# spcl/gemm_hls

Measured on NVIDIA H100. Metric: GFLOP/s at N=16384 K=16384 M=16384 float (Multiply,Add), higher is better.
Workload: dtype tf32 tensor-core multiply, f32 accumulate/storage

## Files before the change

### gemm_hls_b200/csrc/capi.cu

```cuda
#include <algorithm>
#include <chrono>
#include <condition_variable>
#include <cstdlib>
#include <cstring>
#include <functional>
#include <mutex>
#include <string>
#include <thread>
#include <vector>

#include "common.cuh"

namespace mm {

namespace {
thread_local std::string g_last_error = "";
}

void set_error(const std::string &msg) { g_last_error = msg; }
int fail(int code, const std::string &msg) {
  set_error(msg);
  return code;
}

namespace {

struct KnobInfo {
  const char *env;
  int dflt;
};
const KnobInfo kKnobs[MM_TUNE_COUNT] = {
    {"MM_TCGEN05_CTA_GROUP", 2}, {"MM_TCGEN05_BLOCK_N", 256},  {"MM_TCGEN05_STAGES", 0},
    {"MM_TCGEN05_RASTER_ROWS", 2048}, {"MM_TCGEN05_TILE_SYNC", 1}, {"MM_TCGEN05_B_MN", 1},
    {"MM_TCGEN05_L2", 0}, {"MM_TCGEN05_B_OVERLAP", 0}, {"MM_TCGEN05_TMA_STORE", 1},
    {"MM_DMMA_TILE_ROWS", 0}, {"MM_EXPERIMENT_TF32_NO_ROUND", 0}, {"MM_SEMIRING_RING", 1},
};

}

int tuning_validate(int knob, int value) {
  bool ok = false;
  switch (knob) {
    case MM_TUNE_TCGEN05_CTA_GROUP: ok = value == 1 || value == 2; break;
    case MM_TUNE_TCGEN05_BLOCK_N: ok = value == 128 || value == 256; break;
    case MM_TUNE_TCGEN05_STAGES: ok = value == 0 || (value >= 2 && value <= 8); break;
    case MM_TUNE_TCGEN05_RASTER_ROWS: ok = value >= 1; break;
    case MM_TUNE_TCGEN05_L2_POLICY: ok = value >= 0 && value <= 2; break;
    case MM_TUNE_DMMA_TILE_ROWS: ok = value == 0 || value == 64 || value == 128; break;
    case MM_TUNE_TCGEN05_TILE_SYNC:
    case MM_TUNE_TCGEN05_B_MN:
    case MM_TUNE_TCGEN05_B_OVERLAP:
    case MM_TUNE_TCGEN05_TMA_STORE:
    case MM_TUNE_EXPERIMENT_TF32_NO_ROUND:
    case MM_TUNE_SEMIRING_RING: ok = value == 0 || value == 1; break;
    default: return fail(MM_ERR_INVALID, "unknown tuning knob " + std::to_string(knob));
  }
  if (!ok) {
    return fail(MM_ERR_INVALID, std::string("value ") + std::to_string(value) + " is out of range for tuning knob " +
                                    kKnobs[knob].env);
  }
  return MM_OK;
}

Tuning default_tuning() {
  Tuning t;
  for (int i = 0; i < MM_TUNE_COUNT; ++i) {
    t.v[i] = kKnobs[i].dflt;
    const char *e = std::getenv(kKnobs[i].env);
    if (!e || !*e) continue;
    int value;
    if (i == MM_TUNE_TCGEN05_L2_POLICY && (e[0] == 'n' || e[0] == 'f' || e[0] == 'l')) {
      value = e[0] == 'f' ? 1 : (e[0] == 'l' ? 2 : 0);
    } else {
      value = std::atoi(e);
    }
    if (tuning_validate(i, value) == MM_OK) t.v[i] = value;
  }
  return t;
}

}

struct mm_context {
  int device = 0;
  cudaStream_t stream = nullptr;
  cudaStream_t side = nullptr;
  cudaStream_t copy_in = nullptr, copy_out = nullptr;
  std::vector<cudaEvent_t> sync_events;
  cudaEvent_t ev_start = nullptr, ev_stop = nullptr, ev_fork = nullptr, ev_join = nullptr;
  cudaEvent_t ev_slice = nullptr;
  mm::Scratch scratch;
  mm::Scratch staging[3];
  uint64_t staging_gen = 0;
  std::vector<void *> retired;
  bool captured = false;
  mm::Tuning tuning;
  bool profiling = false;
  std::vector<cudaEvent_t> prof_events;
  int prof_calls = 0;
  std::mutex mutex;
};

namespace {

using mm::fail;

bool valid_dtype(int d) { return d >= 0 && d < MM_DTYPE_COUNT; }
bool valid_op(int o) { return o >= 0 && o < MM_OP_COUNT; }

enum Path { kPathTcgen05, kPathDmma, kPathSemiring };

bool tensor_core_dtype(int d) {
  return d == MM_DTYPE_FLOAT || d == MM_DTYPE_HALF || d == MM_DTYPE_BFLOAT16 || d == MM_DTYPE_UINT8;
}

constexpr unsigned kMaxKInt8Tensor = 33024;

Path select_path(int dtype, int map_op, int reduce_op, int flags, unsigned n, unsigned k) {
  const bool dense = (map_op == MM_OP_MULTIPLY && reduce_op == MM_OP_ADD) && !(flags & MM_FLAG_EXACT);
  if (dense && (dtype == MM_DTYPE_FLOAT || dtype == MM_DTYPE_HALF || dtype == MM_DTYPE_BFLOAT16)) return kPathTcgen05;
  if (dense && dtype == MM_DTYPE_UINT8 && k <= kMaxKInt8Tensor) return kPathTcgen05;
  if (dense && dtype == MM_DTYPE_DOUBLE) {
    return ((flags & MM_FLAG_TRANSPOSED_A) && (n % 2 != 0)) ? kPathSemiring : kPathDmma;
  }
  return kPathSemiring;
}

int ensure(mm_context *ctx, mm::Scratch &s, size_t bytes, bool keep_old) {
  if (s.bytes >= bytes) return MM_OK;
  if (s.ptr) {
    if (keep_old) ctx->retired.push_back(s.ptr);
    else cudaFree(s.ptr);
  }
  s.ptr = nullptr;
  s.bytes = 0;
  cudaError_t e = cudaMalloc(&s.ptr, bytes);
  if (e != cudaSuccess) {
    return fail(e == cudaErrorMemoryAllocation ? MM_ERR_NOMEM : MM_ERR_CUDA,
                std::string("cudaMalloc(") + std::to_string(bytes) + "): " + cudaGetErrorString(e));
  }
  s.bytes = bytes;
  return MM_OK;
}

int check_args(int dtype, int map_op, int reduce_op, const void *a, const void *b, const void *c,
               unsigned n, unsigned k, unsigned m) {
  if (!valid_dtype(dtype)) return fail(MM_ERR_INVALID, "unknown MM_DATA_TYPE code");
  if (!valid_op(map_op) || !valid_op(reduce_op)) return fail(MM_ERR_INVALID, "unknown MM_MAP_OP / MM_REDUCE_OP code");
  if (!a || !b || !c) return fail(MM_ERR_INVALID, "null matrix pointer");
  if (n == 0 || k == 0 || m == 0) return fail(MM_ERR_INVALID, "matrix dimensions must be positive");
  const unsigned w = mm_memory_width(dtype);
  if (k % w != 0) {
    return fail(MM_ERR_SHAPE, "K (" + std::to_string(k) + ") must be divisable by the memory width in K (" +
                                  std::to_string(w) + ").");
  }
  if (m % w != 0) {
    return fail(MM_ERR_SHAPE, "M (" + std::to_string(m) + ") must be divisable by the memory width in M (" +
                                  std::to_string(w) + ").");
  }
  return MM_OK;
}

int check_device_alignment(const void *a, const void *b, const void *c) {
  if ((reinterpret_cast<uintptr_t>(a) | reinterpret_cast<uintptr_t>(b) | reinterpret_cast<uintptr_t>(c)) % 16 != 0) {
    return fail(MM_ERR_INVALID, "device matrix pointers must be 16-byte aligned");
  }
  return MM_OK;
}

mm::GemmArgs make_args(mm_context *ctx, const void *a, const void *b, void *c, unsigned n, unsigned k, unsigned m,
                       int flags, cudaStream_t stream) {
  mm::GemmArgs g{a, b, c, n, k, m, flags, stream};
  g.tuning = &ctx->tuning;
  g.side_stream = ctx->side;
  g.ev_fork = ctx->ev_fork;
  g.ev_join = ctx->ev_join;
  return g;
}

mm::GemmBatch make_batch(unsigned batch, int flags) {
  mm::GemmBatch bt;
  bt.count = batch;
  bt.shared_a = (flags & MM_FLAG_BATCH_SHARED_A) != 0;
  bt.shared_b = (flags & MM_FLAG_BATCH_SHARED_B) != 0;
  return bt;
}

int check_batch(unsigned batch, unsigned n, unsigned k, unsigned m) {
  if (batch == 0) return fail(MM_ERR_INVALID, "batch must be positive");
  if (batch > 65535) {
    return fail(MM_ERR_UNSUPPORTED, "batch (" + std::to_string(batch) + ") must not exceed 65535");
  }
  const uint64_t limit = uint64_t(1) << 31;
  if (uint64_t(batch) * n >= limit || uint64_t(batch) * k >= limit || uint64_t(batch) * m >= limit) {
    return fail(MM_ERR_UNSUPPORTED, "batch * N, batch * K and batch * M must be below 2^31");
  }
  return MM_OK;
}

bool overlaps(const void *x, size_t x_bytes, const void *y, size_t y_bytes) {
  const uintptr_t x0 = reinterpret_cast<uintptr_t>(x), y0 = reinterpret_cast<uintptr_t>(y);
  return x0 < y0 + y_bytes && y0 < x0 + x_bytes;
}

int begin_call(mm_context *ctx, cudaStream_t stream, bool profile, cudaStreamCaptureStatus *capture,
               cudaEvent_t **pe) {
  *capture = cudaStreamCaptureStatusNone;
  if (cudaStreamIsCapturing(stream, capture) == cudaSuccess && *capture != cudaStreamCaptureStatusNone) {
    ctx->captured = true;
  }
  *pe = nullptr;
  if (profile && ctx->profiling && ctx->prof_calls < 256) {
    while (ctx->prof_events.size() < size_t(3 * (ctx->prof_calls + 1))) {
      cudaEvent_t e;
      MM_CUDA_TRY(cudaEventCreate(&e));
      ctx->prof_events.push_back(e);
    }
    *pe = &ctx->prof_events[3 * ctx->prof_calls];
    ++ctx->prof_calls;
    MM_CUDA_TRY(cudaEventRecord((*pe)[0], stream));
  }
  return MM_OK;
}

int enqueue_locked(mm_context *ctx, int dtype, int map_op, int reduce_op, int flags, const void *a,
                   const void *b, void *c, unsigned n, unsigned k, unsigned m, cudaStream_t stream,
                   bool dry_run = false, unsigned batch = 1, bool accumulate = false,
                   const mm::AgreeFn *agree = nullptr) {
  mm::GemmArgs g = make_args(ctx, a, b, c, n, k, m, flags, stream);
  g.agree = agree;
  g.batch = make_batch(batch, flags);
  g.dry_run = dry_run;
  g.accumulate = accumulate;
  cudaStreamCaptureStatus capture;
  cudaEvent_t *pe;
  const int rc_begin = begin_call(ctx, stream, !dry_run, &capture, &pe);
  if (rc_begin != MM_OK) return rc_begin;
  if (pe) {
    g.ev_start = pe[0];
    g.ev_prep_done = pe[1];
  }
  int rc_launch = MM_OK;
  switch (select_path(dtype, map_op, reduce_op, flags, n, k)) {
    case kPathTcgen05: {
      const size_t need = mm::tcgen05_scratch_bytes(dtype, n, k, m, flags, ctx->tuning, g.batch);
      if (need > ctx->scratch.bytes && capture != cudaStreamCaptureStatusNone) {
        return fail(MM_ERR_INVALID, batch > 1 ? "the scratch cannot grow during stream capture: call mm_context_reserve_batched() first"
                                              : "the scratch cannot grow during stream capture: call mm_context_reserve() first");
      }
      int rc = ensure(ctx, ctx->scratch, need, ctx->captured);
      if (rc != MM_OK) return rc;
      rc_launch = mm::launch_tcgen05(dtype, g, ctx->scratch.ptr, ctx->scratch.bytes);
      break;
    }
    case kPathDmma:
      if (pe) MM_CUDA_TRY(cudaEventRecord(pe[1], stream));
      rc_launch = accumulate ? mm::launch_dmma_accumulate(g) : mm::launch_dmma(g);
      break;
    case kPathSemiring:
      if (pe) MM_CUDA_TRY(cudaEventRecord(pe[1], stream));
      rc_launch = accumulate ? mm::launch_semiring_accumulate(dtype, map_op, reduce_op, g)
                             : mm::launch_semiring(dtype, map_op, reduce_op, g);
      break;
  }
  if (rc_launch != MM_OK) return rc_launch;
  if (pe) MM_CUDA_TRY(cudaEventRecord(pe[2], stream));
  return MM_OK;
}

void destroy_context(mm_context *ctx) {
  cudaSetDevice(ctx->device);
  if (ctx->stream) cudaStreamSynchronize(ctx->stream);
  if (ctx->side) cudaStreamSynchronize(ctx->side);
  if (ctx->scratch.ptr) cudaFree(ctx->scratch.ptr);
  for (auto &s : ctx->staging) {
    if (s.ptr) cudaFree(s.ptr);
  }
  for (void *p : ctx->retired) cudaFree(p);
  for (auto e : ctx->prof_events) cudaEventDestroy(e);
  for (auto e : ctx->sync_events) cudaEventDestroy(e);
  for (cudaEvent_t e : {ctx->ev_start, ctx->ev_stop, ctx->ev_fork, ctx->ev_join, ctx->ev_slice}) {
    if (e) cudaEventDestroy(e);
  }
  for (cudaStream_t s : {ctx->copy_in, ctx->copy_out, ctx->side, ctx->stream}) {
    if (s) cudaStreamDestroy(s);
  }
  delete ctx;
}

int init_context(mm_context *ctx) {
  MM_CUDA_TRY(cudaStreamCreateWithFlags(&ctx->stream, cudaStreamNonBlocking));
  MM_CUDA_TRY(cudaStreamCreateWithFlags(&ctx->side, cudaStreamNonBlocking));
  MM_CUDA_TRY(cudaStreamCreateWithFlags(&ctx->copy_in, cudaStreamNonBlocking));
  MM_CUDA_TRY(cudaStreamCreateWithFlags(&ctx->copy_out, cudaStreamNonBlocking));
  MM_CUDA_TRY(cudaEventCreate(&ctx->ev_start));
  MM_CUDA_TRY(cudaEventCreate(&ctx->ev_stop));
  MM_CUDA_TRY(cudaEventCreateWithFlags(&ctx->ev_fork, cudaEventDisableTiming));
  MM_CUDA_TRY(cudaEventCreateWithFlags(&ctx->ev_join, cudaEventDisableTiming));
  MM_CUDA_TRY(cudaEventCreateWithFlags(&ctx->ev_slice, cudaEventDisableTiming));
  return MM_OK;
}

struct BPlan {
  unsigned k0 = 0, k1 = 0;
  const void *const *parts_dev = nullptr;
  unsigned parts = 1, part_rows = 0;
  std::vector<cudaEvent_t> peer_slices;
};

struct Pipeline {
  mm_context *ctx;
  int dtype, map_op, reduce_op, flags;
  const unsigned char *a_host;
  const unsigned char *b_host;
  unsigned char *c_host;
  unsigned rows, k, m;
  size_t es;
  Path path;
  unsigned char *da = nullptr, *db = nullptr, *dc = nullptr;

  int upload_b(const BPlan &bp) {
    MM_CUDA_TRY(cudaSetDevice(ctx->device));
    ++ctx->staging_gen;
    int rc;
    if ((rc = ensure(ctx, ctx->staging[0], size_t(rows) * k * es, false)) != MM_OK) return rc;
    if ((rc = ensure(ctx, ctx->staging[1], size_t(k) * m * es, false)) != MM_OK) return rc;
    if ((rc = ensure(ctx, ctx->staging[2], size_t(rows) * m * es, false)) != MM_OK) return rc;
    if (path == kPathTcgen05) {
      rc = ensure(ctx, ctx->scratch, mm::tcgen05_scratch_bytes(dtype, rows, k, m, flags, ctx->tuning), ctx->captured);
      if (rc != MM_OK) return rc;
    }
    da = static_cast<unsigned char *>(ctx->staging[0].ptr);
    db = static_cast<unsigned char *>(ctx->staging[1].ptr);
    dc = static_cast<unsigned char *>(ctx->staging[2].ptr);
    const size_t off = size_t(bp.k0) * m * es, bytes = size_t(bp.k1 - bp.k0) * m * es;
    if (bytes) MM_CUDA_TRY(cudaMemcpyAsync(db + off, b_host + off, bytes, cudaMemcpyHostToDevice, ctx->copy_in));
    MM_CUDA_TRY(cudaEventRecord(ctx->ev_slice, ctx->copy_in));
    return MM_OK;
  }

  int run(const BPlan &bp, double *seconds_device, const mm::AgreeFn *agree = nullptr) {
    const int rc = enqueue_all(bp, agree);
    cudaError_t e = cudaSuccess;
    for (cudaStream_t s : {ctx->copy_in, ctx->side, ctx->stream, ctx->copy_out}) {
      const cudaError_t es_ = cudaStreamSynchronize(s);
      if (e == cudaSuccess) e = es_;
    }
    if (rc != MM_OK) return rc;
    if (e != cudaSuccess) return fail(MM_ERR_CUDA, std::string("host pipeline: ") + cudaGetErrorString(e));
    if (seconds_device) {
      float ms = 0.f;
      MM_CUDA_TRY(cudaEventElapsedTime(&ms, ctx->ev_start, ctx->ev_stop));
      *seconds_device = 1e-3 * ms;
    }
    return MM_OK;
  }

 private:
  int enqueue_all(const BPlan &bp, const mm::AgreeFn *agree) {
    MM_CUDA_TRY(cudaSetDevice(ctx->device));
    const bool ta = (flags & MM_FLAG_TRANSPOSED_A) != 0;
    const mm::Tuning &t = ctx->tuning;
    unsigned chunk_rows = rows;
    if (!ta) {
      const size_t row_bytes = size_t(k) * es;
      size_t cr = std::max<size_t>((rows + 15) / 16, ((size_t(32) << 20) + row_bytes - 1) / row_bytes);
      if (const char *e = std::getenv("MM_HOST_CHUNK_ROWS")) cr = std::max(1, std::atoi(e));
      cr = (cr + 127) / 128 * 128;
      if (cr < rows) chunk_rows = unsigned(cr);
    }
    const unsigned chunks = (rows + chunk_rows - 1) / chunk_rows;
    while (ctx->sync_events.size() < size_t(2 * chunks)) {
      cudaEvent_t e;
      MM_CUDA_TRY(cudaEventCreateWithFlags(&e, cudaEventDisableTiming));
      ctx->sync_events.push_back(e);
    }
    auto ev_a = [&](unsigned i) { return ctx->sync_events[i]; };
    auto ev_c = [&](unsigned i) { return ctx->sync_events[chunks + i]; };

    for (unsigned i = 0; i < chunks; ++i) {
      const size_t r0 = size_t(i) * chunk_rows, nr = std::min<size_t>(chunk_rows, rows - r0);
      if (!ta) {
        MM_CUDA_TRY(cudaMemcpyAsync(da + r0 * k * es, a_host + r0 * k * es, nr * k * es, cudaMemcpyHostToDevice,
                                    ctx->copy_in));
      } else {
        MM_CUDA_TRY(cudaMemcpyAsync(da, a_host, size_t(rows) * k * es, cudaMemcpyHostToDevice, ctx->copy_in));
      }
      MM_CUDA_TRY(cudaEventRecord(ev_a(i), ctx->copy_in));
    }

    MM_CUDA_TRY(cudaStreamWaitEvent(ctx->stream, ctx->ev_slice, 0));
    for (cudaEvent_t e : bp.peer_slices) MM_CUDA_TRY(cudaStreamWaitEvent(ctx->stream, e, 0));
    MM_CUDA_TRY(cudaEventRecord(ctx->ev_start, ctx->stream));
    mm::BSource src;
    src.b = db;
    if (bp.parts_dev != nullptr) {
      src.src = bp.parts_dev;
      src.parts = bp.parts;
      src.part_rows = bp.part_rows;
    }
    int rc = MM_OK;
    mm::PreparedB pb;
    unsigned char *aprep = nullptr;
    mm::HalfScratch hs;
    if (path == kPathTcgen05) {
      hs = mm::tcgen05_half_scratch(ctx->scratch.ptr, ctx->scratch.bytes, dtype, rows, k, m, flags, t);
      if (hs.fits_b) MM_CUDA_TRY(cudaMemsetAsync(hs.fits_b, 1, hs.flag_bytes, ctx->stream));
      rc = mm::tcgen05_prepare_b_async(dtype, src, db, ctx->scratch.ptr, ctx->scratch.bytes, k, m, flags, t, ctx->stream,
                                       ctx->side, ctx->ev_fork, ctx->ev_join, &pb, 1, hs.b, hs.fits_b);
      if (rc != MM_OK) return rc;
      aprep = static_cast<unsigned char *>(ctx->scratch.ptr) + mm::tcgen05_bt_bytes(dtype, k, m, flags, t);
    } else if (bp.parts_dev != nullptr) {
      rc = mm::gather_b_rows(src, db, es, k, m, ctx->stream);
      if (rc != MM_OK) return rc;
    }
    const bool prepare_first = hs.fits_a != nullptr;
    std::vector<const void *> a_ops(chunks);
    auto prepare = [&](unsigned i) -> int {
      const size_t r0 = size_t(i) * chunk_rows, nr = std::min<size_t>(chunk_rows, rows - r0);
      MM_CUDA_TRY(cudaStreamWaitEvent(ctx->stream, ev_a(i), 0));
      if (path != kPathTcgen05) return MM_OK;
      const size_t a_scale = (dtype == MM_DTYPE_FLOAT && (flags & MM_FLAG_TF32X3)) ? 3 : 1;
      return mm::tcgen05_prepare_a(dtype, da + (ta ? 0 : r0 * k * es), aprep + (ta ? 0 : r0 * k * es * a_scale),
                                   unsigned(nr), k, flags, t, &a_ops[i], ctx->stream, 1,
                                   hs.a ? static_cast<unsigned char *>(hs.a) + r0 * k * 2 : nullptr, hs.fits_a);
    };
    auto compute = [&](unsigned i) -> int {
      const size_t r0 = size_t(i) * chunk_rows, nr = std::min<size_t>(chunk_rows, rows - r0);
      const void *a_chunk = da + (ta ? 0 : r0 * k * es);
      void *c_chunk = dc + r0 * m * es;
      int rc1;
      if (path == kPathTcgen05) {
        mm::HalfOperands half = hs.operands();
        if (half.a) half.a = static_cast<const unsigned char *>(half.a) + r0 * k * 2;
        const mm::Tcgen05Counters cnt = mm::tcgen05_counters(ctx->scratch.ptr, ctx->scratch.bytes);
        rc1 = mm::tcgen05_gemm(dtype, a_ops[i], pb.b_op, c_chunk, unsigned(nr), k, m, flags, t, cnt.tile_sync, pb.ready,
                               pb.ready_target, ctx->stream, mm::GemmBatch{}, false, half);
      } else {
        mm::GemmArgs g = make_args(ctx, a_chunk, db, c_chunk, unsigned(nr), k, m, flags, ctx->stream);
        rc1 = (path == kPathDmma) ? mm::launch_dmma(g) : mm::launch_semiring(dtype, map_op, reduce_op, g);
      }
      if (rc1 == MM_OK) MM_CUDA_TRY(cudaEventRecord(ev_c(i), ctx->stream));
      return rc1;
    };
    if (prepare_first) {
      for (unsigned i = 0; i < chunks && rc == MM_OK; ++i) rc = prepare(i);
    }
    if (rc == MM_OK && agree != nullptr) rc = (*agree)(hs.fits_a, ctx->stream);
    for (unsigned i = 0; i < chunks && rc == MM_OK; ++i) {
      if (!prepare_first) rc = prepare(i);
      if (rc == MM_OK) rc = compute(i);
    }
    if (path == kPathTcgen05 && pb.forked) cudaStreamWaitEvent(ctx->stream, ctx->ev_join, 0);
    if (rc != MM_OK) return rc;
    MM_CUDA_TRY(cudaEventRecord(ctx->ev_stop, ctx->stream));

    for (unsigned i = 0; i < chunks; ++i) {
      const size_t r0 = size_t(i) * chunk_rows, nr = std::min<size_t>(chunk_rows, rows - r0);
      MM_CUDA_TRY(cudaStreamWaitEvent(ctx->copy_out, ev_c(i), 0));
      MM_CUDA_TRY(cudaMemcpyAsync(c_host + r0 * m * es, dc + r0 * m * es, nr * m * es, cudaMemcpyDeviceToHost,
                                  ctx->copy_out));
    }
    return MM_OK;
  }
};

std::mutex g_default_mutex;
mm_context *g_default_ctx = nullptr;
mm_multi *g_default_multi = nullptr;

int env_int(const char *name, int fallback) {
  const char *e = std::getenv(name);
  return (e && *e) ? std::atoi(e) : fallback;
}

class HostBarrier {
 public:
  explicit HostBarrier(int n) : n_(n) {}
  void arrive_and_wait() {
    std::unique_lock<std::mutex> lock(m_);
    const int gen = gen_;
    if (++count_ == n_) {
      count_ = 0;
      ++gen_;
      cv_.notify_all();
    } else {
      cv_.wait(lock, [&] { return gen_ != gen; });
    }
  }

 private:
  std::mutex m_;
  std::condition_variable cv_;
  int n_, count_ = 0, gen_ = 0;
};

class FitsAgreement {
 public:
  FitsAgreement(HostBarrier &barrier, int gpus) : barrier_(barrier), fit_(gpus, 1), agreed_(gpus, 0) {}
  mm::AgreeFn agree(int g) {
    return [this, g](unsigned int *fits, cudaStream_t stream) -> int {
      agreed_[g] = 1;
      int rc = MM_OK;
      unsigned int v = 1;
      if (fits != nullptr) {
        cudaError_t e = cudaStreamSynchronize(stream);
        if (e == cudaSuccess) e = cudaMemcpy(&v, fits, sizeof(v), cudaMemcpyDeviceToHost);
        if (e != cudaSuccess) rc = fail(MM_ERR_CUDA, std::string("reading the fits word of A: ") + cudaGetErrorString(e));
      }
      fit_[g] = v != 0u;
      barrier_.arrive_and_wait();
      const bool all = std::all_of(fit_.begin(), fit_.end(), [](int f) { return f != 0; });
      if (rc == MM_OK && fits != nullptr && v != 0u && !all) MM_CUDA_TRY(cudaMemsetAsync(fits, 0, sizeof(v), stream));
      return rc;
    };
  }
  void finish(int g) {
    if (!agreed_[g]) barrier_.arrive_and_wait();
  }

 private:
  HostBarrier &barrier_;
  std::vector<int> fit_;
  std::vector<char> agreed_;
};

}

struct mm_multi {
  std::vector<mm_context *> ctx;
  std::vector<void **> parts_dev;
  bool peer = false;
  std::mutex mutex;
  unsigned n = 0, k = 0, m = 0;
  int dtype = -1;
  std::vector<uint64_t> gen;
  bool executed = false;
};

namespace {

unsigned rows_per_gpu(unsigned n, int g) { return (n + unsigned(g) - 1) / unsigned(g); }

struct Partition {
  unsigned r0, r1;
  unsigned k0, k1;
  unsigned part_rows, parts;
};
Partition partition_for(int gpus, int g, unsigned n, unsigned k, bool sliced_b) {
  Partition p;
  const unsigned per = rows_per_gpu(n, gpus);
  p.r0 = std::min(n, unsigned(g) * per);
  p.r1 = std::min(n, p.r0 + per);
  p.part_rows = sliced_b ? std::max(64u, (rows_per_gpu(k, gpus) + 63u) / 64u * 64u) : k;
  p.parts = sliced_b ? (k + p.part_rows - 1) / p.part_rows : 1;
  if (sliced_b) {
    p.k0 = std::min(k, unsigned(g) * p.part_rows);
    p.k1 = (unsigned(g) >= p.parts) ? p.k0 : std::min(k, p.k0 + p.part_rows);
  } else {
    p.k0 = 0;
    p.k1 = k;
  }
  return p;
}

template <class Fn>
int fan_out(int gpus, Fn fn) {
  std::vector<int> rc(gpus, MM_OK);
  std::vector<std::string> msg(gpus);
  std::vector<std::thread> pool;
  for (int g = 0; g < gpus; ++g) {
    pool.emplace_back([&, g] {
      rc[g] = fn(g);
      if (rc[g] != MM_OK) msg[g] = mm_last_error();
    });
  }
  for (auto &t : pool) t.join();
  for (int g = 0; g < gpus; ++g) {
    if (rc[g] != MM_OK) return fail(rc[g], "GPU " + std::to_string(g) + ": " + msg[g]);
  }
  return MM_OK;
}

int refresh_parts(mm_multi *mu, int g) {
  mm_context *ctx = mu->ctx[g];
  MM_CUDA_TRY(cudaSetDevice(ctx->device));
  std::vector<void *> table(mu->ctx.size());
  for (size_t j = 0; j < mu->ctx.size(); ++j) table[j] = mu->ctx[j]->staging[1].ptr;
  MM_CUDA_TRY(cudaMemcpy(mu->parts_dev[g], table.data(), table.size() * sizeof(void *), cudaMemcpyHostToDevice));
  return MM_OK;
}

int multi_gemm_host_locked(mm_multi *mu, int dtype, int map_op, int reduce_op, int flags, const void *a, const void *b,
                           void *c, unsigned n, unsigned k, unsigned m, double *seconds_device) {
  if (flags & MM_FLAG_TRANSPOSED_A) {
    return fail(MM_ERR_UNSUPPORTED, "the row-block split over GPUs needs row-major A (MM_TRANSPOSED_A is set)");
  }
  const int G = int(mu->ctx.size());
  const size_t es = mm_dtype_size(dtype);
  std::vector<Pipeline> pipes(G);
  std::vector<BPlan> plans(G);
  std::vector<double> dev_s(G, 0.0);
  HostBarrier barrier(G);
  FitsAgreement fits(barrier, G);
  int rc = fan_out(G, [&](int g) -> int {
    const Partition part = partition_for(G, g, n, k, mu->peer);
    const unsigned r0 = part.r0, r1 = part.r1;
    Pipeline &p = pipes[g];
    p = Pipeline{mu->ctx[g], dtype, map_op, reduce_op, flags,
                 static_cast<const unsigned char *>(a) + size_t(r0) * k * es, static_cast<const unsigned char *>(b),
                 static_cast<unsigned char *>(c) + size_t(r0) * m * es, r1 - r0, k, m, es,
                 select_path(dtype, map_op, reduce_op, flags, std::max(1u, r1 - r0), k)};
    BPlan &bp = plans[g];
    bp.k0 = part.k0;
    bp.k1 = part.k1;
    if (mu->peer) {
      bp.parts = part.parts;
      bp.part_rows = part.part_rows;
      bp.parts_dev = mu->parts_dev[g];
    }
    std::lock_guard<std::mutex> lock(mu->ctx[g]->mutex);
    if (p.rows == 0) p.rows = 1, p.a_host = static_cast<const unsigned char *>(a), p.c_host = nullptr;
    int rc1 = p.upload_b(bp);
    barrier.arrive_and_wait();
    int rc2 = (rc1 == MM_OK && mu->peer) ? refresh_parts(mu, g) : MM_OK;
    if (mu->peer) {
      for (int j = 0; j < G; ++j) {
        if (j != g) bp.peer_slices.push_back(mu->ctx[j]->ev_slice);
      }
    }
    barrier.arrive_and_wait();
    const mm::AgreeFn agree = fits.agree(g);
    int rc3 = MM_OK;
    if (rc1 == MM_OK && rc2 == MM_OK && r1 > r0) {
      rc3 = p.run(bp, &dev_s[g], &agree);
    } else {
      cudaSetDevice(mu->ctx[g]->device);
      cudaStreamSynchronize(mu->ctx[g]->copy_in);
    }
    fits.finish(g);
    barrier.arrive_and_wait();
    return rc1 != MM_OK ? rc1 : (rc2 != MM_OK ? rc2 : rc3);
  });
  if (rc != MM_OK) return rc;
  if (seconds_device) *seconds_device = *std::max_element(dev_s.begin(), dev_s.end());
  return MM_OK;
}

void clear_resident(mm_multi *mu) {
  mu->n = mu->k = mu->m = 0;
  mu->dtype = -1;
  mu->gen.clear();
  mu->executed = false;
}

int check_resident(mm_multi *mu, const char *entry, int dtype, unsigned n, unsigned k, unsigned m) {
  if (mu->dtype != dtype || mu->n != n || mu->k != k || mu->m != m) {
    return fail(MM_ERR_INVALID, std::string(entry) + ": no matching mm_multi_upload (type or sizes differ)");
  }
  for (size_t g = 0; g < mu->ctx.size(); ++g) {
    std::lock_guard<std::mutex> lock(mu->ctx[g]->mutex);
    if (mu->ctx[g]->staging_gen != mu->gen[g]) {
      return fail(MM_ERR_INVALID, std::string(entry) + ": no matching mm_multi_upload (GPU " + std::to_string(g) +
                                      "'s buffers were reused by another call since)");
    }
  }
  return MM_OK;
}

int create_multi(int n_gpus, const int *devices, mm_multi **out) {
  mm_multi *mu = new mm_multi();
  auto cleanup = [&](int rc) {
    const std::string msg = mm_last_error();
    mm_multi_destroy(mu);
    mm::set_error(msg);
    return rc;
  };
  for (int g = 0; g < n_gpus; ++g) {
    mm_context *c = nullptr;
    const int rc = mm_context_create(devices ? devices[g] : g, &c);
    if (rc != MM_OK) return cleanup(rc);
    mu->ctx.push_back(c);
  }
  mu->peer = n_gpus > 1;
  for (int g = 0; g < n_gpus && mu->peer; ++g) {
    for (int j = 0; j < n_gpus; ++j) {
      if (mu->ctx[j]->device == mu->ctx[g]->device) continue;
      int can = 0;
      if (cudaDeviceCanAccessPeer(&can, mu->ctx[g]->device, mu->ctx[j]->device) != cudaSuccess || !can) mu->peer = false;
    }
  }
  for (int g = 0; g < n_gpus; ++g) {
    if (cudaSetDevice(mu->ctx[g]->device) != cudaSuccess) return cleanup(fail(MM_ERR_CUDA, "cudaSetDevice failed"));
    for (int j = 0; j < n_gpus && mu->peer; ++j) {
      if (mu->ctx[j]->device == mu->ctx[g]->device) continue;
      const cudaError_t e = cudaDeviceEnablePeerAccess(mu->ctx[j]->device, 0);
      if (e == cudaErrorPeerAccessAlreadyEnabled) cudaGetLastError();
      else if (e != cudaSuccess) mu->peer = false;
    }
    void **table = nullptr;
    if (cudaMalloc(&table, sizeof(void *) * size_t(n_gpus)) != cudaSuccess) {
      return cleanup(fail(MM_ERR_NOMEM, "cudaMalloc of the slice table failed"));
    }
    mu->parts_dev.push_back(table);
  }
  *out = mu;
  return MM_OK;
}

int kernel_execute(mm_context *ctx, int dtype, int map_op, int reduce_op, int flags, const void *a, const void *b,
                   void *c, unsigned n, unsigned k, unsigned m, double *seconds_device, double *seconds_wall,
                   const mm::AgreeFn *agree) {
  if (!ctx) return fail(MM_ERR_INVALID, "null context");
  int rc = check_args(dtype, map_op, reduce_op, a, b, c, n, k, m);
  if (rc != MM_OK) return rc;
  if ((rc = check_device_alignment(a, b, c)) != MM_OK) return rc;
  std::lock_guard<std::mutex> lock(ctx->mutex);
  MM_CUDA_TRY(cudaSetDevice(ctx->device));
  rc = enqueue_locked(ctx, dtype, map_op, reduce_op, flags, a, b, c, n, k, m, ctx->stream, true);
  if (rc != MM_OK) return rc;
  const auto t0 = std::chrono::high_resolution_clock::now();
  MM_CUDA_TRY(cudaEventRecord(ctx->ev_start, ctx->stream));
  rc = enqueue_locked(ctx, dtype, map_op, reduce_op, flags, a, b, c, n, k, m, ctx->stream, false, 1, false, agree);
  if (rc != MM_OK) {
    cudaStreamSynchronize(ctx->stream);
    return rc;
  }
  MM_CUDA_TRY(cudaEventRecord(ctx->ev_stop, ctx->stream));
  MM_CUDA_TRY(cudaEventSynchronize(ctx->ev_stop));
  const auto t1 = std::chrono::high_resolution_clock::now();
  float ms = 0.f;
  MM_CUDA_TRY(cudaEventElapsedTime(&ms, ctx->ev_start, ctx->ev_stop));
  if (seconds_device) *seconds_device = 1e-3 * ms;
  if (seconds_wall) *seconds_wall = std::chrono::duration<double>(t1 - t0).count();
  return MM_OK;
}

}

extern "C" {

const char *mm_last_error(void) { return mm::g_last_error.c_str(); }

int mm_version(void) { return 203; }

size_t mm_dtype_size(int dtype) {
  switch (dtype) {
    case MM_DTYPE_HALF: return 2;
    case MM_DTYPE_FLOAT: return 4;
    case MM_DTYPE_DOUBLE: return 8;
    case MM_DTYPE_INT32: return 4;
    case MM_DTYPE_UINT32: return 4;
    case MM_DTYPE_UINT8: return 1;
    case MM_DTYPE_BFLOAT16: return 2;
  }
  return 0;
}

unsigned mm_memory_width(int dtype) {
  const size_t s = mm_dtype_size(dtype);
  return s ? static_cast<unsigned>(64 / s) : 0;
}

int mm_context_create(int device, mm_context **out) {
  if (!out) return fail(MM_ERR_INVALID, "null output pointer");
  *out = nullptr;
  int count = 0;
  cudaError_t e = cudaGetDeviceCount(&count);
  if (e != cudaSuccess || count == 0) {
    return fail(MM_ERR_CUDA, std::string("no CUDA device available: ") +
                                 (e != cudaSuccess ? cudaGetErrorString(e) : "device count is 0"));
  }
  if (device < 0 || device >= count) return fail(MM_ERR_INVALID, "device ordinal out of range");
  MM_CUDA_TRY(cudaSetDevice(device));
  cudaDeviceProp prop;
  MM_CUDA_TRY(cudaGetDeviceProperties(&prop, device));
  if (prop.major != 9 || prop.minor != 0) {
    return fail(MM_ERR_UNSUPPORTED, std::string("libmm_b200 is built for sm_90a only; device is sm_") +
                                        std::to_string(prop.major) + std::to_string(prop.minor));
  }
  mm_context *ctx = new mm_context();
  ctx->device = device;
  ctx->tuning = mm::default_tuning();
  const int rc = init_context(ctx);
  if (rc != MM_OK) {
    const std::string msg = mm_last_error();
    destroy_context(ctx);
    mm::set_error(msg);
    return rc;
  }
  *out = ctx;
  return MM_OK;
}

int mm_context_destroy(mm_context *ctx) {
  if (!ctx) return MM_OK;
  destroy_context(ctx);
  return MM_OK;
}

int mm_context_set_tuning(mm_context *ctx, int knob, int value) {
  if (!ctx) return fail(MM_ERR_INVALID, "null context");
  const int rc = mm::tuning_validate(knob, value);
  if (rc != MM_OK) return rc;
  std::lock_guard<std::mutex> lock(ctx->mutex);
  ctx->tuning.v[knob] = value;
  return MM_OK;
}

int mm_context_get_tuning(mm_context *ctx, int knob, int *value) {
  if (!ctx || !value) return fail(MM_ERR_INVALID, "null argument");
  if (knob < 0 || knob >= MM_TUNE_COUNT) return fail(MM_ERR_INVALID, "unknown tuning knob " + std::to_string(knob));
  std::lock_guard<std::mutex> lock(ctx->mutex);
  *value = ctx->tuning.v[knob];
  return MM_OK;
}

int mm_context_reserve(mm_context *ctx, int dtype, int flags, unsigned n, unsigned k, unsigned m) {
  if (!ctx) return fail(MM_ERR_INVALID, "null context");
  if (!valid_dtype(dtype)) return fail(MM_ERR_INVALID, "unknown MM_DATA_TYPE code");
  std::lock_guard<std::mutex> lock(ctx->mutex);
  MM_CUDA_TRY(cudaSetDevice(ctx->device));
  if (!tensor_core_dtype(dtype)) return MM_OK;
  return ensure(ctx, ctx->scratch, mm::tcgen05_scratch_bytes(dtype, n, k, m, flags & ~MM_FLAG_EXACT, ctx->tuning),
                ctx->captured);
}

int mm_context_reserve_batched(mm_context *ctx, int dtype, int flags, unsigned n, unsigned k, unsigned m,
                               unsigned batch) {
  if (!ctx) return fail(MM_ERR_INVALID, "null context");
  if (!valid_dtype(dtype)) return fail(MM_ERR_INVALID, "unknown MM_DATA_TYPE code");
  int rc = check_batch(batch, n, k, m);
  if (rc != MM_OK) return rc;
  std::lock_guard<std::mutex> lock(ctx->mutex);
  MM_CUDA_TRY(cudaSetDevice(ctx->device));
  if (!tensor_core_dtype(dtype)) return MM_OK;
  const int f = flags & ~MM_FLAG_EXACT;
  return ensure(ctx, ctx->scratch, mm::tcgen05_scratch_bytes(dtype, n, k, m, f, ctx->tuning, make_batch(batch, f)),
                ctx->captured);
}

int mm_buffer_alloc(mm_context *ctx, size_t bytes, void **device_ptr) {
  if (!ctx || !device_ptr) return fail(MM_ERR_INVALID, "null argument");
  *device_ptr = nullptr;
  MM_CUDA_TRY(cudaSetDevice(ctx->device));
  cudaError_t e = cudaMalloc(device_ptr, bytes ? bytes : 1);
  if (e != cudaSuccess) {
    return fail(e == cudaErrorMemoryAllocation ? MM_ERR_NOMEM : MM_ERR_CUDA,
                std::string("cudaMalloc: ") + cudaGetErrorString(e));
  }
  return MM_OK;
}

int mm_buffer_free(mm_context *ctx, void *device_ptr) {
  if (!ctx) return fail(MM_ERR_INVALID, "null context");
  MM_CUDA_TRY(cudaSetDevice(ctx->device));
  MM_CUDA_TRY(cudaFree(device_ptr));
  return MM_OK;
}

int mm_copy_to_device(mm_context *ctx, void *device_dst, const void *host_src, size_t bytes) {
  if (!ctx || !device_dst || !host_src) return fail(MM_ERR_INVALID, "null argument");
  std::lock_guard<std::mutex> lock(ctx->mutex);
  MM_CUDA_TRY(cudaSetDevice(ctx->device));
  MM_CUDA_TRY(cudaMemcpyAsync(device_dst, host_src, bytes, cudaMemcpyHostToDevice, ctx->stream));
  MM_CUDA_TRY(cudaStreamSynchronize(ctx->stream));
  return MM_OK;
}

int mm_copy_to_host(mm_context *ctx, void *host_dst, const void *device_src, size_t bytes) {
  if (!ctx || !host_dst || !device_src) return fail(MM_ERR_INVALID, "null argument");
  std::lock_guard<std::mutex> lock(ctx->mutex);
  MM_CUDA_TRY(cudaSetDevice(ctx->device));
  MM_CUDA_TRY(cudaMemcpyAsync(host_dst, device_src, bytes, cudaMemcpyDeviceToHost, ctx->stream));
  MM_CUDA_TRY(cudaStreamSynchronize(ctx->stream));
  return MM_OK;
}

int mm_kernel_enqueue(mm_context *ctx, int dtype, int map_op, int reduce_op, int flags,
                      const void *a, const void *b, void *c, unsigned n, unsigned k, unsigned m,
                      void *cuda_stream) {
  if (!ctx) return fail(MM_ERR_INVALID, "null context");
  int rc = check_args(dtype, map_op, reduce_op, a, b, c, n, k, m);
  if (rc != MM_OK) return rc;
  if ((rc = check_device_alignment(a, b, c)) != MM_OK) return rc;
  std::lock_guard<std::mutex> lock(ctx->mutex);
  MM_CUDA_TRY(cudaSetDevice(ctx->device));
  cudaStream_t s = cuda_stream ? static_cast<cudaStream_t>(cuda_stream) : ctx->stream;
  return enqueue_locked(ctx, dtype, map_op, reduce_op, flags, a, b, c, n, k, m, s);
}

int mm_kernel_enqueue_batched(mm_context *ctx, int dtype, int map_op, int reduce_op, int flags, const void *a,
                              const void *b, void *c, unsigned n, unsigned k, unsigned m, unsigned batch,
                              void *cuda_stream) {
  if (!ctx) return fail(MM_ERR_INVALID, "null context");
  int rc = check_args(dtype, map_op, reduce_op, a, b, c, n, k, m);
  if (rc != MM_OK) return rc;
  if ((rc = check_batch(batch, n, k, m)) != MM_OK) return rc;
  if ((rc = check_device_alignment(a, b, c)) != MM_OK) return rc;
  std::lock_guard<std::mutex> lock(ctx->mutex);
  MM_CUDA_TRY(cudaSetDevice(ctx->device));
  cudaStream_t s = cuda_stream ? static_cast<cudaStream_t>(cuda_stream) : ctx->stream;
  return enqueue_locked(ctx, dtype, map_op, reduce_op, flags, a, b, c, n, k, m, s, false, batch);
}

int mm_kernel_enqueue_accumulate(mm_context *ctx, int dtype, int map_op, int reduce_op, int flags, const void *a,
                                 const void *b, void *c, unsigned n, unsigned k, unsigned m, unsigned batch,
                                 void *cuda_stream) {
  if (!ctx) return fail(MM_ERR_INVALID, "null context");
  int rc = check_args(dtype, map_op, reduce_op, a, b, c, n, k, m);
  if (rc != MM_OK) return rc;
  if ((rc = check_batch(batch, n, k, m)) != MM_OK) return rc;
  if ((rc = check_device_alignment(a, b, c)) != MM_OK) return rc;
  const size_t es = mm_dtype_size(dtype);
  const mm::GemmBatch bt = make_batch(batch, flags);
  if (overlaps(c, size_t(batch) * n * m * es, a, size_t(bt.a_copies()) * n * k * es) ||
      overlaps(c, size_t(batch) * n * m * es, b, size_t(bt.b_copies()) * k * m * es)) {
    return fail(MM_ERR_INVALID, "C must not overlap A or B in an accumulating call");
  }
  std::lock_guard<std::mutex> lock(ctx->mutex);
  MM_CUDA_TRY(cudaSetDevice(ctx->device));
  cudaStream_t s = cuda_stream ? static_cast<cudaStream_t>(cuda_stream) : ctx->stream;
  return enqueue_locked(ctx, dtype, map_op, reduce_op, flags, a, b, c, n, k, m, s, false, batch,
                        true);
}

int mm_kernel_enqueue_witness(mm_context *ctx, int dtype, int map_op, int reduce_op, int flags, const void *a,
                              const void *b, void *c, unsigned *w, unsigned n, unsigned k, unsigned m, unsigned batch,
                              void *cuda_stream) {
  if (!ctx) return fail(MM_ERR_INVALID, "null context");
  int rc = check_args(dtype, map_op, reduce_op, a, b, c, n, k, m);
  if (rc != MM_OK) return rc;
  if ((rc = check_batch(batch, n, k, m)) != MM_OK) return rc;
  if ((rc = check_device_alignment(a, b, c)) != MM_OK) return rc;
  if (!w) return fail(MM_ERR_INVALID, "null witness pointer");
  if (reinterpret_cast<uintptr_t>(w) % 16 != 0) return fail(MM_ERR_INVALID, "the witness pointer must be 16-byte aligned");
  if (reduce_op != MM_OP_MIN && reduce_op != MM_OP_MAX) {
    return fail(MM_ERR_INVALID, "witnesses exist for the Min and Max reduces only");
  }
  std::lock_guard<std::mutex> lock(ctx->mutex);
  MM_CUDA_TRY(cudaSetDevice(ctx->device));
  cudaStream_t s = cuda_stream ? static_cast<cudaStream_t>(cuda_stream) : ctx->stream;
  mm::GemmArgs g = make_args(ctx, a, b, c, n, k, m, flags, s);
  g.batch = make_batch(batch, flags);
  cudaStreamCaptureStatus capture;
  cudaEvent_t *pe;
  if ((rc = begin_call(ctx, s, true, &capture, &pe)) != MM_OK) return rc;
  if (pe) MM_CUDA_TRY(cudaEventRecord(pe[1], s));
  if ((rc = mm::launch_semiring_witness(dtype, map_op, reduce_op, g, w)) != MM_OK) return rc;
  if (pe) MM_CUDA_TRY(cudaEventRecord(pe[2], s));
  return MM_OK;
}

int mm_kernel_execute(mm_context *ctx, int dtype, int map_op, int reduce_op, int flags,
                      const void *a, const void *b, void *c, unsigned n, unsigned k, unsigned m,
                      double *seconds_device, double *seconds_wall) {
  return kernel_execute(ctx, dtype, map_op, reduce_op, flags, a, b, c, n, k, m, seconds_device, seconds_wall, nullptr);
}

int mm_context_set_profiling(mm_context *ctx, int enable) {
  if (!ctx) return fail(MM_ERR_INVALID, "null context");
  std::lock_guard<std::mutex> lock(ctx->mutex);
  ctx->profiling = enable != 0;
  ctx->prof_calls = 0;
  return MM_OK;
}

int mm_context_profile_read(mm_context *ctx, double *prep_sum, double *main_sum, int *calls) {
  if (!ctx) return fail(MM_ERR_INVALID, "null context");
  std::lock_guard<std::mutex> lock(ctx->mutex);
  MM_CUDA_TRY(cudaSetDevice(ctx->device));
  double prep = 0.0, main_s = 0.0;
  for (int i = 0; i < ctx->prof_calls; ++i) {
    cudaEvent_t *e = &ctx->prof_events[3 * i];
    MM_CUDA_TRY(cudaEventSynchronize(e[2]));
    float ms_prep = 0.f, ms_main = 0.f;
    MM_CUDA_TRY(cudaEventElapsedTime(&ms_prep, e[0], e[1]));
    MM_CUDA_TRY(cudaEventElapsedTime(&ms_main, e[1], e[2]));
    prep += 1e-3 * ms_prep;
    main_s += 1e-3 * ms_main;
  }
  if (prep_sum) *prep_sum = prep;
  if (main_sum) *main_sum = main_s;
  if (calls) *calls = ctx->prof_calls;
  ctx->prof_calls = 0;
  return MM_OK;
}

int mm_kernel_launch_count(int dtype, int map_op, int reduce_op, int flags) {
  if (!valid_dtype(dtype) || !valid_op(map_op) || !valid_op(reduce_op)) return -1;
  const mm::Tuning t = mm::default_tuning();
  switch (select_path(dtype, map_op, reduce_op, flags, 2, 64)) {
    case kPathTcgen05:
      return 1 + (mm::tcgen05_b_in_place(dtype, flags, t) ? 0 : 1) +
             ((dtype == MM_DTYPE_FLOAT || (flags & MM_FLAG_TRANSPOSED_A)) ? 1 : 0);
    case kPathDmma: return 1;
    case kPathSemiring: return 1;
  }
  return -1;
}

const char *mm_kernel_path(int dtype, int map_op, int reduce_op, int flags) {
  if (!valid_dtype(dtype) || !valid_op(map_op) || !valid_op(reduce_op)) return "invalid";
  switch (select_path(dtype, map_op, reduce_op, flags, 2, 64)) {
    case kPathTcgen05:
      if (dtype == MM_DTYPE_BFLOAT16) return "wgmma_bf16";
      return dtype == MM_DTYPE_FLOAT ? "wgmma_tf32" : (dtype == MM_DTYPE_UINT8 ? "wgmma_i8" : "wgmma_f16");
    case kPathDmma: return "dmma_f64";
    case kPathSemiring: return "semiring_simt";
  }
  return "invalid";
}

int mm_gemm_host(mm_context *ctx, int dtype, int map_op, int reduce_op, int flags, const void *a,
                 const void *b, void *c, unsigned n, unsigned k, unsigned m, double *seconds_device,
                 double *seconds_wall) {
  int rc = check_args(dtype, map_op, reduce_op, a, b, c, n, k, m);
  if (rc != MM_OK) return rc;
  if (!ctx) {
    const bool split = env_int("MM_NUM_GPUS", 1) > 1 && !(flags & MM_FLAG_TRANSPOSED_A);
    {
      std::lock_guard<std::mutex> lock(g_default_mutex);
      if (split && !g_default_multi) rc = mm_multi_create(env_int("MM_NUM_GPUS", 1), nullptr, &g_default_multi);
      if (!split && !g_default_ctx) rc = mm_context_create(env_int("MM_DEVICE", 0), &g_default_ctx);
      if (rc != MM_OK) return rc;
    }
    if (split) {
      return mm_multi_gemm_host(g_default_multi, dtype, map_op, reduce_op, flags, a, b, c, n, k, m, seconds_device,
                                seconds_wall);
    }
    ctx = g_default_ctx;
  }
  const auto t0 = std::chrono::high_resolution_clock::now();
  std::lock_guard<std::mutex> lock(ctx->mutex);
  Pipeline p{ctx, dtype, map_op, reduce_op, flags, static_cast<const unsigned char *>(a),
             static_cast<const unsigned char *>(b), static_cast<unsigned char *>(c), n, k, m, mm_dtype_size(dtype),
             select_path(dtype, map_op, reduce_op, flags, n, k)};
  BPlan bp;
  bp.k0 = 0;
  bp.k1 = k;
  rc = p.upload_b(bp);
  if (rc == MM_OK) {
    rc = p.run(bp, seconds_device);
  } else {
    cudaStreamSynchronize(ctx->copy_in);
  }
  if (rc != MM_OK) return rc;
  if (seconds_wall) {
    *seconds_wall = std::chrono::duration<double>(std::chrono::high_resolution_clock::now() - t0).count();
  }
  return MM_OK;
}


int mm_multi_create(int n_gpus, const int *devices, mm_multi **out) {
  if (!out) return fail(MM_ERR_INVALID, "null output pointer");
  *out = nullptr;
  if (n_gpus < 1) return fail(MM_ERR_INVALID, "mm_multi_create needs at least one device");
  int count = 0;
  cudaError_t e = cudaGetDeviceCount(&count);
  if (e != cudaSuccess || count == 0) {
    return fail(MM_ERR_CUDA, std::string("no CUDA device available: ") +
                                 (e != cudaSuccess ? cudaGetErrorString(e) : "device count is 0"));
  }
  if (!devices && n_gpus > count) {
    return fail(MM_ERR_INVALID, "mm_multi_create: " + std::to_string(n_gpus) + " devices requested, " +
                                    std::to_string(count) + " visible");
  }
  return create_multi(n_gpus, devices, out);
}

int mm_multi_destroy(mm_multi *mu) {
  if (!mu) return MM_OK;
  for (size_t g = 0; g < mu->ctx.size(); ++g) {
    if (g < mu->parts_dev.size() && mu->parts_dev[g]) {
      cudaSetDevice(mu->ctx[g]->device);
      cudaFree(mu->parts_dev[g]);
    }
  }
  for (mm_context *c : mu->ctx) destroy_context(c);
  delete mu;
  return MM_OK;
}

int mm_multi_device_count(const mm_multi *mu) { return mu ? int(mu->ctx.size()) : 0; }

mm_context *mm_multi_context(mm_multi *mu, int index) {
  if (!mu || index < 0 || index >= int(mu->ctx.size())) return nullptr;
  return mu->ctx[index];
}

int mm_multi_peer_access(const mm_multi *mu) { return (mu && mu->peer) ? 1 : 0; }

int mm_multi_partition(int n_gpus, int index, unsigned n, unsigned k, unsigned *row_begin, unsigned *row_end,
                       unsigned *b_row_begin, unsigned *b_row_end) {
  if (n_gpus < 1 || index < 0 || index >= n_gpus) return fail(MM_ERR_INVALID, "mm_multi_partition: bad device count / index");
  const Partition p = partition_for(n_gpus, index, n, k, n_gpus > 1);
  if (row_begin) *row_begin = p.r0;
  if (row_end) *row_end = p.r1;
  if (b_row_begin) *b_row_begin = p.k0;
  if (b_row_end) *b_row_end = p.k1;
  return MM_OK;
}

int mm_multi_gemm_host(mm_multi *mu, int dtype, int map_op, int reduce_op, int flags, const void *a, const void *b,
                       void *c, unsigned n, unsigned k, unsigned m, double *seconds_device, double *seconds_wall) {
  if (!mu) return fail(MM_ERR_INVALID, "null multi-GPU context");
  int rc = check_args(dtype, map_op, reduce_op, a, b, c, n, k, m);
  if (rc != MM_OK) return rc;
  const auto t0 = std::chrono::high_resolution_clock::now();
  std::lock_guard<std::mutex> lock(mu->mutex);
  rc = multi_gemm_host_locked(mu, dtype, map_op, reduce_op, flags, a, b, c, n, k, m, seconds_device);
  if (rc != MM_OK) return rc;
  if (seconds_wall) {
    *seconds_wall = std::chrono::duration<double>(std::chrono::high_resolution_clock::now() - t0).count();
  }
  return MM_OK;
}

int mm_multi_upload(mm_multi *mu, int dtype, int flags, const void *a, const void *b, unsigned n, unsigned k,
                    unsigned m) {
  if (!mu) return fail(MM_ERR_INVALID, "null multi-GPU context");
  std::lock_guard<std::mutex> lock(mu->mutex);
  clear_resident(mu);
  int rc = check_args(dtype, MM_OP_MULTIPLY, MM_OP_ADD, a, b, a , n, k, m);
  if (rc != MM_OK) return rc;
  if (flags & MM_FLAG_TRANSPOSED_A) {
    return fail(MM_ERR_UNSUPPORTED, "the row-block split over GPUs needs row-major A (MM_TRANSPOSED_A is set)");
  }
  const int G = int(mu->ctx.size());
  const size_t es = mm_dtype_size(dtype);
  std::vector<uint64_t> gen(G, 0);
  HostBarrier barrier(G);
  rc = fan_out(G, [&](int g) -> int {
    mm_context *ctx = mu->ctx[g];
    std::lock_guard<std::mutex> ctx_lock(ctx->mutex);
    gen[g] = ++ctx->staging_gen;
    const Partition part = partition_for(G, g, n, k, mu->peer);
    const unsigned r0 = part.r0, r1 = part.r1, part_rows = part.part_rows, parts = part.parts;
    const unsigned rows = std::max(1u, r1 - r0);
    auto body = [&]() -> int {
      MM_CUDA_TRY(cudaSetDevice(ctx->device));
      int r;
      if ((r = ensure(ctx, ctx->staging[0], size_t(rows) * k * es, false)) != MM_OK) return r;
      if ((r = ensure(ctx, ctx->staging[1], size_t(k) * m * es, false)) != MM_OK) return r;
      if ((r = ensure(ctx, ctx->staging[2], size_t(rows) * m * es, false)) != MM_OK) return r;
      unsigned char *db = static_cast<unsigned char *>(ctx->staging[1].ptr);
      const unsigned k0 = part.k0, k1 = part.k1;
      const size_t off = size_t(k0) * m * es;
      if (k1 > k0) {
        MM_CUDA_TRY(cudaMemcpyAsync(db + off, static_cast<const unsigned char *>(b) + off, size_t(k1 - k0) * m * es,
                                    cudaMemcpyHostToDevice, ctx->copy_in));
      }
      MM_CUDA_TRY(cudaEventRecord(ctx->ev_slice, ctx->copy_in));
      if (r1 > r0) {
        MM_CUDA_TRY(cudaMemcpyAsync(ctx->staging[0].ptr, static_cast<const unsigned char *>(a) + size_t(r0) * k * es,
                                    size_t(r1 - r0) * k * es, cudaMemcpyHostToDevice, ctx->copy_in));
      }
      return MM_OK;
    };
    const int rc1 = body();
    barrier.arrive_and_wait();
    int rc2 = MM_OK;
    if (rc1 == MM_OK && mu->peer) {
      rc2 = refresh_parts(mu, g);
    }
    barrier.arrive_and_wait();
    if (rc1 == MM_OK && rc2 == MM_OK && mu->peer) {
      auto gather = [&]() -> int {
        MM_CUDA_TRY(cudaStreamWaitEvent(ctx->stream, ctx->ev_slice, 0));
        for (int j = 0; j < G; ++j) {
          if (j != g) MM_CUDA_TRY(cudaStreamWaitEvent(ctx->stream, mu->ctx[j]->ev_slice, 0));
        }
        mm::BSource src;
        src.src = mu->parts_dev[g];
        src.parts = parts;
        src.part_rows = part_rows;
        return mm::gather_b_rows(src, ctx->staging[1].ptr, es, k, m, ctx->stream);
      };
      rc2 = gather();
    }
    cudaSetDevice(ctx->device);
    cudaStreamSynchronize(ctx->copy_in);
    cudaStreamSynchronize(ctx->stream);
    barrier.arrive_and_wait();
    return rc1 != MM_OK ? rc1 : rc2;
  });
  if (rc != MM_OK) return rc;
  mu->n = n;
  mu->k = k;
  mu->m = m;
  mu->dtype = dtype;
  mu->gen = gen;
  return MM_OK;
}

int mm_multi_execute(mm_multi *mu, int dtype, int map_op, int reduce_op, int flags, unsigned n, unsigned k, unsigned m,
                     double *seconds_device, double *seconds_wall) {
  if (!mu) return fail(MM_ERR_INVALID, "null multi-GPU context");
  if (!valid_dtype(dtype) || !valid_op(map_op) || !valid_op(reduce_op)) return fail(MM_ERR_INVALID, "unknown type / operator code");
  std::lock_guard<std::mutex> lock(mu->mutex);
  int rc = check_resident(mu, "mm_multi_execute", dtype, n, k, m);
  if (rc != MM_OK) return rc;
  mu->executed = false;
  const int G = int(mu->ctx.size());
  std::vector<double> dev_s(G, 0.0);
  const auto t0 = std::chrono::high_resolution_clock::now();
  HostBarrier barrier(G);
  FitsAgreement fits(barrier, G);
  rc = fan_out(G, [&](int g) -> int {
    const Partition part = partition_for(G, g, n, k, mu->peer);
    const unsigned r0 = part.r0, r1 = part.r1;
    int r = MM_OK;
    if (r1 > r0) {
      mm_context *ctx = mu->ctx[g];
      const mm::AgreeFn agree = fits.agree(g);
      r = kernel_execute(ctx, dtype, map_op, reduce_op, flags, ctx->staging[0].ptr, ctx->staging[1].ptr,
                         ctx->staging[2].ptr, r1 - r0, k, m, &dev_s[g], nullptr, &agree);
    }
    fits.finish(g);
    return r;
  });
  if (rc != MM_OK) return rc;
  mu->executed = true;
  if (seconds_device) *seconds_device = *std::max_element(dev_s.begin(), dev_s.end());
  if (seconds_wall) {
    *seconds_wall = std::chrono::duration<double>(std::chrono::high_resolution_clock::now() - t0).count();
  }
  return MM_OK;
}

int mm_multi_download(mm_multi *mu, int dtype, void *c, unsigned n, unsigned m) {
  if (!mu || !c) return fail(MM_ERR_INVALID, "null argument");
  std::lock_guard<std::mutex> lock(mu->mutex);
  const int rc = check_resident(mu, "mm_multi_download", dtype, n, mu->k, m);
  if (rc != MM_OK) return rc;
  if (!mu->executed) return fail(MM_ERR_INVALID, "mm_multi_download: no mm_multi_execute since the last upload");
  const int G = int(mu->ctx.size());
  const size_t es = mm_dtype_size(dtype);
  return fan_out(G, [&](int g) -> int {
    const Partition part = partition_for(G, g, n, 64, false);
    const unsigned r0 = part.r0, r1 = part.r1;
    if (r1 == r0) return MM_OK;
    mm_context *ctx = mu->ctx[g];
    return mm_copy_to_host(ctx, static_cast<unsigned char *>(c) + size_t(r0) * m * es, ctx->staging[2].ptr,
                           size_t(r1 - r0) * m * es);
  });
}

}
```

### gemm_hls_b200/csrc/common.cuh

```cuda
#pragma once

#include <cuda_runtime.h>

#include <cstdio>
#include <functional>
#include <string>

#include "../../include/mm_b200.h"

namespace mm {

using AgreeFn = std::function<int(unsigned int *fits_a, cudaStream_t stream)>;

void set_error(const std::string &msg);
int fail(int code, const std::string &msg);

#define MM_CUDA_TRY(expr)                                                                  \
  do {                                                                                     \
    cudaError_t err__ = (expr);                                                            \
    if (err__ != cudaSuccess) {                                                            \
      return ::mm::fail(MM_ERR_CUDA, std::string(#expr) + ": " + cudaGetErrorString(err__)); \
    }                                                                                      \
  } while (0)

inline unsigned ceil_div(unsigned a, unsigned b) { return (a + b - 1) / b; }

struct Scratch {
  void *ptr = nullptr;
  size_t bytes = 0;
};

struct Tuning {
  int v[MM_TUNE_COUNT];
  int cta_group() const { return v[MM_TUNE_TCGEN05_CTA_GROUP]; }
  int block_n() const { return v[MM_TUNE_TCGEN05_BLOCK_N]; }
  int stages() const { return v[MM_TUNE_TCGEN05_STAGES]; }
  int raster_rows() const { return v[MM_TUNE_TCGEN05_RASTER_ROWS]; }
  bool tile_sync() const { return v[MM_TUNE_TCGEN05_TILE_SYNC] != 0; }
  bool b_mn() const { return v[MM_TUNE_TCGEN05_B_MN] != 0; }
  int l2_policy() const { return v[MM_TUNE_TCGEN05_L2_POLICY]; }
  int b_overlap() const { return v[MM_TUNE_TCGEN05_B_OVERLAP]; }
  bool tma_store() const { return v[MM_TUNE_TCGEN05_TMA_STORE] != 0; }
  int dmma_tile_rows() const { return v[MM_TUNE_DMMA_TILE_ROWS]; }
  bool tf32_no_round() const { return v[MM_TUNE_EXPERIMENT_TF32_NO_ROUND] != 0; }
  bool semiring_ring() const { return v[MM_TUNE_SEMIRING_RING] != 0; }
};
Tuning default_tuning();
int tuning_validate(int knob, int value);

struct GemmBatch {
  unsigned count = 1;
  bool shared_a = false, shared_b = false;
  unsigned a_copies() const { return shared_a ? 1u : count; }
  unsigned b_copies() const { return shared_b ? 1u : count; }
};

struct GemmArgs {
  const void *a;
  const void *b;
  void *c;
  unsigned n, k, m;
  int flags;
  cudaStream_t stream;
  const Tuning *tuning = nullptr;
  GemmBatch batch;
  cudaStream_t side_stream = nullptr;
  cudaEvent_t ev_fork = nullptr, ev_join = nullptr;
  cudaEvent_t ev_start = nullptr;
  cudaEvent_t ev_prep_done = nullptr;
  bool dry_run = false;
  bool accumulate = false;
  const AgreeFn *agree = nullptr;
};

int launch_semiring(int dtype, int map_op, int reduce_op, const GemmArgs &args);
int launch_semiring_witness(int dtype, int map_op, int reduce_op, const GemmArgs &args, unsigned *w);
int launch_semiring_accumulate(int dtype, int map_op, int reduce_op, const GemmArgs &args);

size_t tcgen05_scratch_bytes(int dtype, unsigned n, unsigned k, unsigned m, int flags, const Tuning &t,
                             const GemmBatch &batch = GemmBatch{});
size_t tcgen05_bt_bytes(int dtype, unsigned k, unsigned m, int flags, const Tuning &t,
                        unsigned b_copies = 1);
int launch_tcgen05(int dtype, const GemmArgs &args, void *scratch, size_t scratch_bytes);
struct HalfOperands {
  const void *a = nullptr, *b = nullptr;
  const unsigned int *fits_a = nullptr, *fits_b = nullptr;
};
struct HalfScratch {
  void *a = nullptr, *b = nullptr;
  unsigned int *fits_a = nullptr, *fits_b = nullptr;
  size_t flag_bytes = 0;
  HalfOperands operands() const { return HalfOperands{a, b, fits_a, fits_b}; }
};
HalfScratch tcgen05_half_scratch(void *scratch, size_t scratch_bytes, int dtype, unsigned n, unsigned k, unsigned m,
                                 int flags, const Tuning &t, const GemmBatch &batch = GemmBatch{});
bool tcgen05_b_mn(int dtype, int flags, const Tuning &t);
bool tcgen05_b_in_place(int dtype, int flags, const Tuning &t);

struct BSource {
  const void *b = nullptr;
  const void *const *src = nullptr;
  unsigned parts = 1;
  unsigned part_rows = 0;
};
struct Tcgen05Counters {
  unsigned int *tile_sync;
  unsigned int *b_ready;
};
Tcgen05Counters tcgen05_counters(void *scratch, size_t scratch_bytes);
int tcgen05_prepare_b(int dtype, const BSource &src, void *bt, unsigned k, unsigned m, int flags, const Tuning &t,
                      const void **b_op, unsigned int *ready, unsigned *ready_target, cudaStream_t stream,
                      unsigned copies = 1, void *bt16 = nullptr, unsigned int *fits = nullptr);
struct PreparedB {
  const void *b_op = nullptr;
  const unsigned int *ready = nullptr;
  unsigned ready_target = 0;
  bool forked = false;
};
int tcgen05_prepare_b_async(int dtype, const BSource &src, void *local_b, void *scratch, size_t scratch_bytes,
                            unsigned k, unsigned m, int flags, const Tuning &t, cudaStream_t stream, cudaStream_t side,
                            cudaEvent_t ev_fork, cudaEvent_t ev_join, PreparedB *out, unsigned copies = 1,
                            void *bt16 = nullptr, unsigned int *fits = nullptr);
int tcgen05_prepare_a(int dtype, const void *a, void *aprep, unsigned rows, unsigned k, int flags, const Tuning &t,
                      const void **a_op, cudaStream_t stream, unsigned copies = 1, void *aprep16 = nullptr,
                      unsigned int *fits = nullptr);
int tcgen05_gemm(int dtype, const void *a_op, const void *b_op, void *c, unsigned rows, unsigned k, unsigned m,
                 int flags, const Tuning &t, unsigned int *tile_sync, const unsigned int *b_ready,
                 unsigned b_ready_target, cudaStream_t stream, const GemmBatch &batch = GemmBatch{},
                 bool accumulate = false, const HalfOperands &half = HalfOperands{});
constexpr size_t kTcgen05TailBytes = 256 + 64 * 1024;
int gather_b_rows(const BSource &src, void *dst, size_t elem_bytes, unsigned k, unsigned m, cudaStream_t stream);

int launch_dmma(const GemmArgs &args);
int launch_dmma_accumulate(const GemmArgs &args);

}
```

### gemm_hls_b200/csrc/gemm_tcgen05.cu

```cuda
#include <cuda.h>
#include <cuda_fp16.h>
#include <cuda_runtime.h>

#include <algorithm>
#include <cstdlib>
#include <cstring>
#include <vector>

#include "common.cuh"
#include "fits_half.h"
#include "gemm_wgmma.cuh"
#include "ptx_sm90.cuh"
#include "tma_host.cuh"

namespace mm {
namespace {

__device__ __forceinline__ float round_tf32(float x) {
  uint32_t r;
  asm("cvt.rna.tf32.f32 %0, %1;" : "=r"(r) : "f"(x));
  const bool overflowed = (r & 0x7FFFFFFFu) == 0x7F800000u && (__float_as_uint(x) & 0x7FFFFFFFu) != 0x7F800000u;
  return __uint_as_float(overflowed ? ((r & 0x80000000u) | 0x7F7FE000u) : r);
}


__device__ __forceinline__ uint32_t half2_bits(float lo, float hi) {
  const __half2 h = __floats2half2_rn(lo, hi);
  return *reinterpret_cast<const uint32_t *>(&h);
}

template <bool HALF>
__global__ void __launch_bounds__(256)
round_tf32_kernel(const float4 *__restrict__ src, float4 *__restrict__ dst, size_t count4, uint2 *__restrict__ dst16,
                  unsigned int *__restrict__ fits) {
  src += size_t(blockIdx.y) * count4;
  dst += size_t(blockIdx.y) * count4;
  const size_t stride = size_t(gridDim.x) * blockDim.x;
  bool fit = true;
  for (size_t i = size_t(blockIdx.x) * blockDim.x + threadIdx.x; i < count4; i += stride) {
    float4 v = src[i];
    v.x = round_tf32(v.x);
    v.y = round_tf32(v.y);
    v.z = round_tf32(v.z);
    v.w = round_tf32(v.w);
    dst[i] = v;
    if constexpr (HALF) {
      dst16[size_t(blockIdx.y) * count4 + i] = make_uint2(half2_bits(v.x, v.y), half2_bits(v.z, v.w));
      fit = fit && tf32_fits_half(__float_as_uint(v.x)) && tf32_fits_half(__float_as_uint(v.y)) &&
            tf32_fits_half(__float_as_uint(v.z)) && tf32_fits_half(__float_as_uint(v.w));
    }
  }
  if constexpr (HALF) {
    if (__syncthreads_or(!fit) && threadIdx.x == 0) fits[blockIdx.y] = 0u;
  }
}

constexpr int PREP_THREADS = 512;
constexpr int PREP_WARPS = PREP_THREADS / 32;
constexpr int PANEL_ROWS = 64;
constexpr int PANEL_ROW_SLOTS = PANEL_ROWS / PREP_WARPS;

template <bool ROUND>
__device__ __forceinline__ uint4 prep_vec(uint4 v) {
  if (ROUND) {
    v.x = __float_as_uint(round_tf32(__uint_as_float(v.x)));
    v.y = __float_as_uint(round_tf32(__uint_as_float(v.y)));
    v.z = __float_as_uint(round_tf32(__uint_as_float(v.z)));
    v.w = __float_as_uint(round_tf32(__uint_as_float(v.w)));
  }
  return v;
}

template <bool ROUND>
__global__ void __launch_bounds__(PREP_THREADS)
prep_b_panels_kernel(const uint4 *__restrict__ single, const uint4 *const *__restrict__ parts, uint32_t part_rows,
                     uint4 *__restrict__ dst, uint32_t k, uint32_t row_v, uint32_t panel_v,
                     unsigned int *__restrict__ ready) {
  const uint32_t warp = threadIdx.x / 32, lane = threadIdx.x % 32;
  const uint32_t panels = (row_v + panel_v - 1) / panel_v;
  const uint32_t items_per_panel = (k + PANEL_ROWS - 1) / PANEL_ROWS;
  const uint32_t items = panels * items_per_panel;
  for (uint32_t item = blockIdx.x; item < items; item += gridDim.x) {
    const uint32_t panel = item / items_per_panel;
    const uint32_t r0 = (item - panel * items_per_panel) * PANEL_ROWS;
    const uint32_t v0 = panel * panel_v;
    const uint32_t w = min(panel_v, row_v - v0);
    for (uint32_t c0 = 0; c0 < w; c0 += 64) {
      uint4 buf[PANEL_ROW_SLOTS][2];
      bool live[PANEL_ROW_SLOTS][2];
#pragma unroll
      for (int u = 0; u < PANEL_ROW_SLOTS; ++u) {
        const uint32_t r = r0 + warp + u * PREP_WARPS;
        const uint4 *src = single;
        if (parts != nullptr && r < k) src = parts[r / part_rows];
#pragma unroll
        for (int h = 0; h < 2; ++h) {
          const uint32_t c = c0 + lane + 32 * h;
          const size_t off = size_t(r) * row_v + v0 + c;
          live[u][h] = (r < k) && (c < w) && (src + off != static_cast<const uint4 *>(dst) + off);
          if (live[u][h]) buf[u][h] = src[off];
        }
      }
#pragma unroll
      for (int u = 0; u < PANEL_ROW_SLOTS; ++u) {
        const uint32_t r = r0 + warp + u * PREP_WARPS;
#pragma unroll
        for (int h = 0; h < 2; ++h) {
          const uint32_t c = c0 + lane + 32 * h;
          if (live[u][h]) dst[size_t(r) * row_v + v0 + c] = prep_vec<ROUND>(buf[u][h]);
        }
      }
    }
    if (ready != nullptr) {
      __threadfence();
      __syncthreads();
      if (threadIdx.x == 0) atomicAdd(ready + panel, 1u);
    }
  }
}

template <typename T, bool ROUND>
__device__ __forceinline__ T prep_value(T x) {
  return x;
}
template <>
__device__ __forceinline__ float prep_value<float, true>(float x) {
  return round_tf32(x);
}

template <typename T, bool ROUND>
__global__ void __launch_bounds__(256)
transpose_prep_kernel(const T *__restrict__ src, T *__restrict__ dst, uint32_t src_rows,
                      uint32_t src_cols, __half *__restrict__ dst16, unsigned int *__restrict__ fits) {
  constexpr int TILE = 64;
  constexpr int PAD = (sizeof(T) >= 4) ? 1 : 2;
  __shared__ T tile[TILE][TILE + PAD];
  src += size_t(blockIdx.z) * src_rows * src_cols;
  dst += size_t(blockIdx.z) * src_rows * src_cols;
  const uint32_t c0 = blockIdx.x * TILE;
  const uint32_t r0 = blockIdx.y * TILE;
  const int x = threadIdx.x % TILE;
  const int y = threadIdx.x / TILE;
#pragma unroll 4
  for (int i = y; i < TILE; i += 4) {
    const uint32_t r = r0 + i, c = c0 + x;
    if (r < src_rows && c < src_cols) tile[i][x] = prep_value<T, ROUND>(src[size_t(r) * src_cols + c]);
  }
  __syncthreads();
  bool fit = true;
#pragma unroll 4
  for (int i = y; i < TILE; i += 4) {
    const uint32_t c = c0 + i, r = r0 + x;
    if (c < src_cols && r < src_rows) {
      const T v = tile[x][i];
      dst[size_t(c) * src_rows + r] = v;
      if constexpr (ROUND) {
        dst16[size_t(blockIdx.z) * src_rows * src_cols + size_t(c) * src_rows + r] = __float2half_rn(v);
        fit = fit && tf32_fits_half(__float_as_uint(v));
      }
    }
  }
  if constexpr (ROUND) {
    if (__syncthreads_or(!fit) && threadIdx.x == 0) fits[blockIdx.z] = 0u;
  }
}

constexpr int SPLIT_BLOCK = 16;

__device__ __forceinline__ void split_tf32(float x, float &hi, float &lo) {
  hi = round_tf32(x);
  lo = isinf(x) ? 0.0f : round_tf32(x - hi);
}

__device__ __forceinline__ float finite_or_zero(float hi) { return isinf(hi) ? 0.0f : hi; }

__global__ void __launch_bounds__(256)
split3_rows_kernel(const float4 *__restrict__ src, float4 *__restrict__ dst, size_t rows, uint32_t k) {
  const size_t k4 = k / 4;
  const size_t total = rows * k4;
  const size_t stride = size_t(gridDim.x) * blockDim.x;
  for (size_t i = size_t(blockIdx.x) * blockDim.x + threadIdx.x; i < total; i += stride) {
    const size_t r = i / k4;
    const uint32_t c4 = uint32_t(i - r * k4);
    const uint32_t blk = c4 / (SPLIT_BLOCK / 4), in = c4 % (SPLIT_BLOCK / 4);
    const float4 v = src[i];
    float4 hi, lo;
    split_tf32(v.x, hi.x, lo.x);
    split_tf32(v.y, hi.y, lo.y);
    split_tf32(v.z, hi.z, lo.z);
    split_tf32(v.w, hi.w, lo.w);
    float4 *row = dst + r * (3 * k4) + size_t(blk) * (3 * SPLIT_BLOCK / 4) + in;
    row[0] = hi;
    row[SPLIT_BLOCK / 4] = make_float4(finite_or_zero(hi.x), finite_or_zero(hi.y), finite_or_zero(hi.z),
                                       finite_or_zero(hi.w));
    row[2 * SPLIT_BLOCK / 4] = lo;
  }
}

template <bool B_ORDER>
__global__ void __launch_bounds__(256)
split3_transpose_kernel(const float *__restrict__ src, float *__restrict__ dst, uint32_t src_rows,
                        uint32_t src_cols) {
  constexpr int TILE = 64;
  __shared__ float tile[TILE][TILE + 1];
  src += size_t(blockIdx.z) * src_rows * src_cols;
  dst += size_t(blockIdx.z) * src_rows * src_cols * 3;
  const uint32_t c0 = blockIdx.x * TILE;
  const uint32_t r0 = blockIdx.y * TILE;
  const int x = threadIdx.x % TILE;
  const int y = threadIdx.x / TILE;
#pragma unroll 4
  for (int i = y; i < TILE; i += 4) {
    const uint32_t r = r0 + i, c = c0 + x;
    if (r < src_rows && c < src_cols) tile[i][x] = src[size_t(r) * src_cols + c];
  }
  __syncthreads();
#pragma unroll 4
  for (int i = y; i < TILE; i += 4) {
    const uint32_t c = c0 + i, r = r0 + x;
    if (c < src_cols && r < src_rows) {
      float hi, lo;
      split_tf32(tile[x][i], hi, lo);
      float *out = dst + size_t(c) * (3 * size_t(src_rows)) + size_t(r / SPLIT_BLOCK) * (3 * SPLIT_BLOCK) +
                   (r % SPLIT_BLOCK);
      out[0] = hi;
      out[SPLIT_BLOCK] = B_ORDER ? lo : finite_or_zero(hi);
      out[2 * SPLIT_BLOCK] = B_ORDER ? finite_or_zero(hi) : lo;
    }
  }
}


size_t align_up(size_t x, size_t a) { return (x + a - 1) / a * a; }

template <typename T, bool ROUND>
void launch_transpose(const void *src, void *dst, uint32_t src_rows, uint32_t src_cols, cudaStream_t stream,
                      unsigned copies, void *dst16 = nullptr, unsigned int *fits = nullptr) {
  dim3 grid((src_cols + 63) / 64, (src_rows + 63) / 64, copies);
  transpose_prep_kernel<T, ROUND><<<grid, 256, 0, stream>>>(static_cast<const T *>(src), static_cast<T *>(dst),
                                                           src_rows, src_cols, static_cast<__half *>(dst16), fits);
}

int launch_round(const void *src, void *dst, size_t count4, unsigned copies, void *dst16, unsigned int *fits,
                 cudaStream_t stream) {
  const int blocks = int(std::min<size_t>((count4 + 255) / 256, size_t(num_sms()) * 16));
  const dim3 grid(std::max(blocks, 1), copies);
  const float4 *s = static_cast<const float4 *>(src);
  float4 *d = static_cast<float4 *>(dst);
  if (dst16 != nullptr) {
    MM_CUDA_TRY(cudaFuncSetAttribute(round_tf32_kernel<true>, cudaFuncAttributePreferredSharedMemoryCarveout,
                                     cudaSharedmemCarveoutMaxShared));
    round_tf32_kernel<true><<<grid, 256, 0, stream>>>(s, d, count4, static_cast<uint2 *>(dst16), fits);
  } else {
    MM_CUDA_TRY(cudaFuncSetAttribute(round_tf32_kernel<false>, cudaFuncAttributePreferredSharedMemoryCarveout,
                                     cudaSharedmemCarveoutMaxShared));
    round_tf32_kernel<false><<<grid, 256, 0, stream>>>(s, d, count4, nullptr, nullptr);
  }
  return MM_OK;
}

bool split3(int dtype, int flags) { return dtype == MM_DTYPE_FLOAT && (flags & MM_FLAG_TF32X3); }

int launch_panels(bool round, const BSource &src, void *dst, size_t elem_bytes, unsigned k, unsigned m,
                  unsigned panel_cols, unsigned int *ready, int grid, cudaStream_t stream) {
  const uint32_t row_v = uint32_t(size_t(m) * elem_bytes / 16);
  const uint32_t panel_v = uint32_t(size_t(panel_cols) * elem_bytes / 16);
  const uint4 *single = static_cast<const uint4 *>(src.b);
  const uint4 *const *parts = reinterpret_cast<const uint4 *const *>(src.src);
  if (round) {
    prep_b_panels_kernel<true><<<grid, PREP_THREADS, 0, stream>>>(single, parts, src.part_rows, static_cast<uint4 *>(dst),
                                                                 k, row_v, panel_v, ready);
  } else {
    prep_b_panels_kernel<false><<<grid, PREP_THREADS, 0, stream>>>(single, parts, src.part_rows, static_cast<uint4 *>(dst),
                                                                  k, row_v, panel_v, ready);
  }
  MM_CUDA_TRY(cudaGetLastError());
  return MM_OK;
}

}

constexpr size_t TILE_SYNC_BYTES = 256;
constexpr size_t B_READY_BYTES = 64 * 1024;
constexpr size_t TAIL_BYTES = TILE_SYNC_BYTES + B_READY_BYTES;
static_assert(TAIL_BYTES == kTcgen05TailBytes, "common.cuh and gemm_tcgen05.cu disagree on the scratch tail");

Tcgen05Counters tcgen05_counters(void *scratch, size_t scratch_bytes) {
  unsigned char *tail = static_cast<unsigned char *>(scratch) + scratch_bytes;
  return Tcgen05Counters{reinterpret_cast<unsigned int *>(tail - TILE_SYNC_BYTES),
                         reinterpret_cast<unsigned int *>(tail - TAIL_BYTES)};
}

bool tcgen05_b_mn(int, int, const Tuning &) { return false; }

bool tcgen05_b_in_place(int dtype, int flags, const Tuning &t) {
  return tcgen05_b_mn(dtype, flags, t) && (dtype == MM_DTYPE_HALF || dtype == MM_DTYPE_UINT8 || t.tf32_no_round());
}

bool half_copies(int dtype, int flags, const Tuning &t) {
  return dtype == MM_DTYPE_FLOAT && !split3(dtype, flags) && !t.tf32_no_round();
}

size_t b_copy_bytes(int dtype, unsigned k, unsigned m, int flags, unsigned b_copies) {
  return align_up(size_t(b_copies) * m * k * elem_bytes(dtype) * (split3(dtype, flags) ? 3 : 1), 1024);
}
size_t a_copy_bytes(int dtype, unsigned n, unsigned k, int flags, unsigned a_copies) {
  if (dtype != MM_DTYPE_FLOAT && !(flags & MM_FLAG_TRANSPOSED_A)) return 0;
  return align_up(size_t(a_copies) * n * k * elem_bytes(dtype) * (split3(dtype, flags) ? 3 : 1), 1024);
}
size_t fits_bytes(const GemmBatch &batch) {
  return align_up(size_t(batch.a_copies() + batch.b_copies()) * sizeof(unsigned int), 1024);
}

size_t tcgen05_bt_bytes(int dtype, unsigned k, unsigned m, int flags, const Tuning &t, unsigned b_copies) {
  if (tcgen05_b_in_place(dtype, flags, t)) return 0;
  const size_t fp16 = half_copies(dtype, flags, t) ? align_up(size_t(b_copies) * m * k * 2, 1024) : 0;
  return b_copy_bytes(dtype, k, m, flags, b_copies) + fp16;
}

size_t tcgen05_scratch_bytes(int dtype, unsigned n, unsigned k, unsigned m, int flags, const Tuning &t,
                             const GemmBatch &batch) {
  size_t bytes = TAIL_BYTES + tcgen05_bt_bytes(dtype, k, m, flags, t, batch.b_copies());
  bytes += a_copy_bytes(dtype, n, k, flags, batch.a_copies());
  if (half_copies(dtype, flags, t)) bytes += align_up(size_t(batch.a_copies()) * n * k * 2, 1024) + fits_bytes(batch);
  return bytes;
}

HalfScratch tcgen05_half_scratch(void *scratch, size_t scratch_bytes, int dtype, unsigned n, unsigned k, unsigned m,
                                 int flags, const Tuning &t, const GemmBatch &batch) {
  HalfScratch h;
  if (!half_copies(dtype, flags, t)) return h;
  unsigned char *sp = static_cast<unsigned char *>(scratch);
  const size_t bt = tcgen05_bt_bytes(dtype, k, m, flags, t, batch.b_copies());
  h.b = sp + b_copy_bytes(dtype, k, m, flags, batch.b_copies());
  h.a = sp + bt + a_copy_bytes(dtype, n, k, flags, batch.a_copies());
  h.flag_bytes = fits_bytes(batch);
  h.fits_b = reinterpret_cast<unsigned int *>(sp + scratch_bytes - TAIL_BYTES - h.flag_bytes);
  h.fits_a = h.fits_b + batch.b_copies();
  return h;
}

int gather_b_rows(const BSource &src, void *dst, size_t elem_bytes, unsigned k, unsigned m, cudaStream_t stream) {
  return launch_panels(false, src, dst, elem_bytes, k, m, unsigned(1024 / elem_bytes), nullptr,
                       num_sms() * 2, stream);
}

int tcgen05_prepare_b(int dtype, const BSource &src, void *bt, unsigned k, unsigned m, int flags, const Tuning &t,
                      const void **b_op, unsigned int *ready, unsigned *ready_target, cudaStream_t stream,
                      unsigned copies, void *bt16, unsigned int *fits) {
  *b_op = bt;
  if (ready_target) *ready_target = 0;
  const bool parts = src.src != nullptr;
  const size_t eb = elem_bytes(dtype);
  if (tcgen05_b_mn(dtype, flags, t)) {
    if (copies != 1) return fail(MM_ERR_UNSUPPORTED, "batched calls need the K-major B copy");
    const bool in_place = tcgen05_b_in_place(dtype, flags, t);
    if (in_place && !parts) {
      *b_op = src.b;
      return MM_OK;
    }
    if (!in_place && !parts && ready == nullptr) {
      const int rc = launch_round(src.b, bt, size_t(k) * m / 4, 1, nullptr, nullptr, stream);
      if (rc != MM_OK) return rc;
      MM_CUDA_TRY(cudaGetLastError());
      return MM_OK;
    }
    const unsigned panel_cols = unsigned(t.block_n());
    const unsigned panels = ceil_div(m, panel_cols);
    const bool publish = ready != nullptr && panels <= B_READY_BYTES / sizeof(unsigned int);
    if (publish && ready_target) *ready_target = ceil_div(k, PANEL_ROWS);
    const int grid = publish ? num_sms() : num_sms() * 2;
    MM_CUDA_TRY(cudaFuncSetAttribute(prep_b_panels_kernel<true>, cudaFuncAttributePreferredSharedMemoryCarveout,
                                     cudaSharedmemCarveoutMaxShared));
    MM_CUDA_TRY(cudaFuncSetAttribute(prep_b_panels_kernel<false>, cudaFuncAttributePreferredSharedMemoryCarveout,
                                     cudaSharedmemCarveoutMaxShared));
    return launch_panels(!in_place, src, bt, eb, k, m, panel_cols, publish ? ready : nullptr, grid, stream);
  }
  const void *b = src.b;
  if (parts) return fail(MM_ERR_UNSUPPORTED, "row-sliced B needs the MN-major B path (gather it first)");
  if (split3(dtype, flags)) {
    dim3 grid((m + 63) / 64, (k + 63) / 64, copies);
    split3_transpose_kernel<true><<<grid, 256, 0, stream>>>(static_cast<const float *>(b), static_cast<float *>(bt), k, m);
  } else if (dtype == MM_DTYPE_FLOAT) {
    if (t.tf32_no_round()) {
      launch_transpose<float, false>(b, bt, k, m, stream, copies);
    } else {
      launch_transpose<float, true>(b, bt, k, m, stream, copies, bt16, fits);
    }
  } else if (dtype == MM_DTYPE_UINT8) {
    launch_transpose<unsigned char, false>(b, bt, k, m, stream, copies);
  } else {
    launch_transpose<__half, false>(b, bt, k, m, stream, copies);
  }
  MM_CUDA_TRY(cudaGetLastError());
  return MM_OK;
}

int tcgen05_prepare_a(int dtype, const void *a, void *aprep, unsigned rows, unsigned k, int flags, const Tuning &t,
                      const void **a_op, cudaStream_t stream, unsigned copies, void *aprep16, unsigned int *fits) {
  const bool transposed = (flags & MM_FLAG_TRANSPOSED_A) != 0;
  const size_t all_rows = size_t(copies) * rows;
  *a_op = a;
  if (split3(dtype, flags)) {
    if (transposed) {
      dim3 grid((rows + 63) / 64, (k + 63) / 64, copies);
      split3_transpose_kernel<false><<<grid, 256, 0, stream>>>(static_cast<const float *>(a),
                                                              static_cast<float *>(aprep), k, rows);
    } else {
      const size_t total4 = all_rows * k / 4;
      const int blocks = int(std::min<size_t>((total4 + 255) / 256, size_t(num_sms()) * 16));
      split3_rows_kernel<<<blocks, 256, 0, stream>>>(static_cast<const float4 *>(a),
                                                    static_cast<float4 *>(aprep), all_rows, k);
    }
    *a_op = aprep;
  } else if (dtype == MM_DTYPE_FLOAT) {
    if (transposed) {
      if (t.tf32_no_round()) {
        launch_transpose<float, false>(a, aprep, k, rows, stream, copies);
      } else {
        launch_transpose<float, true>(a, aprep, k, rows, stream, copies, aprep16, fits);
      }
      *a_op = aprep;
    } else if (!t.tf32_no_round()) {
      const int rc = launch_round(a, aprep, size_t(rows) * k / 4, copies, aprep16, fits, stream);
      if (rc != MM_OK) return rc;
      *a_op = aprep;
    }
  } else if (transposed) {
    if (dtype == MM_DTYPE_UINT8) launch_transpose<unsigned char, false>(a, aprep, k, rows, stream, copies);
    else launch_transpose<__half, false>(a, aprep, k, rows, stream, copies);
    *a_op = aprep;
  }
  MM_CUDA_TRY(cudaGetLastError());
  return MM_OK;
}

namespace {
int gemm_dispatch(int dtype, const void *a_op, const void *b_op, void *c, unsigned rows, unsigned k, unsigned m,
                  int flags, const Tuning &t, unsigned int *tile_sync, const unsigned int *b_ready,
                  unsigned b_ready_target, bool attributes_only, cudaStream_t stream, const GemmBatch &batch,
                  bool accumulate = false, const HalfOperands &half = HalfOperands{}) {
  if (accumulate) {
    if (split3(dtype, flags)) k *= 3;
    return wgmma_accumulate_gemm(dtype, a_op, b_op, c, rows, k, m, t, tile_sync, b_ready, b_ready_target,
                                 attributes_only, stream, batch, half);
  }
  if (dtype == MM_DTYPE_BFLOAT16) {
    return wgmma_bf16_gemm(a_op, b_op, c, rows, k, m, t, tile_sync, b_ready, b_ready_target, attributes_only, stream,
                           batch);
  }
  if (split3(dtype, flags)) k *= 3;
  CUtensorMap maps[5];
  LaunchPlan plan;
  const int rc = plan_gemm(dtype, a_op, b_op, c, rows, k, m, t, tile_sync, b_ready, b_ready_target, attributes_only,
                           stream, batch, half, maps, &plan);
  if (rc != MM_OK) return rc;
  const int cg = t.cta_group(), bn = t.block_n();
  if (dtype == MM_DTYPE_UINT8) return dispatch_variant<ptx::KIND_I8, unsigned char>(cg, bn, plan);
  return dtype == MM_DTYPE_FLOAT ? dispatch_variant<ptx::KIND_TF32, float>(cg, bn, plan)
                                 : dispatch_variant<ptx::KIND_F16, __half>(cg, bn, plan);
}

}

int tcgen05_gemm(int dtype, const void *a_op, const void *b_op, void *c, unsigned rows, unsigned k, unsigned m,
                 int flags, const Tuning &t, unsigned int *tile_sync, const unsigned int *b_ready,
                 unsigned b_ready_target, cudaStream_t stream, const GemmBatch &batch, bool accumulate,
                 const HalfOperands &half) {
  return gemm_dispatch(dtype, a_op, b_op, c, rows, k, m, flags, t, tile_sync, b_ready, b_ready_target, false, stream,
                       batch, accumulate, half);
}

int tcgen05_prepare_b_async(int dtype, const BSource &src, void *local_b, void *scratch, size_t scratch_bytes,
                            unsigned k, unsigned m, int flags, const Tuning &t, cudaStream_t stream, cudaStream_t side,
                            cudaEvent_t ev_fork, cudaEvent_t ev_join, PreparedB *out, unsigned copies, void *bt16,
                            unsigned int *fits) {
  *out = PreparedB{};
  const bool in_place = tcgen05_b_in_place(dtype, flags, t);
  const bool parts = src.src != nullptr;
  if (copies != 1) {
    if (parts) return fail(MM_ERR_UNSUPPORTED, "batched calls take B from one array");
    return tcgen05_prepare_b(dtype, src, scratch, k, m, flags, t, &out->b_op, nullptr, nullptr, stream, copies, bt16,
                             fits);
  }
  if (parts && !tcgen05_b_mn(dtype, flags, t)) {
    int rc = gather_b_rows(src, local_b, elem_bytes(dtype), k, m, stream);
    if (rc != MM_OK) return rc;
    BSource whole;
    whole.b = local_b;
    return tcgen05_prepare_b(dtype, whole, scratch, k, m, flags, t, &out->b_op, nullptr, nullptr, stream, 1, bt16, fits);
  }
  void *bt = in_place ? local_b : scratch;
  const Tcgen05Counters cnt = tcgen05_counters(scratch, scratch_bytes);
  const unsigned panels = ceil_div(m, unsigned(t.block_n()));
  const bool overlap = side != nullptr && t.b_overlap() != 0 && tcgen05_b_mn(dtype, flags, t) && (!in_place || parts) &&
                       panels <= B_READY_BYTES / sizeof(unsigned int);
  if (!overlap) return tcgen05_prepare_b(dtype, src, bt, k, m, flags, t, &out->b_op, nullptr, nullptr, stream, 1, bt16, fits);
  MM_CUDA_TRY(cudaMemsetAsync(cnt.b_ready, 0, panels * sizeof(unsigned int), stream));
  MM_CUDA_TRY(cudaEventRecord(ev_fork, stream));
  MM_CUDA_TRY(cudaStreamWaitEvent(side, ev_fork, 0));
  const int rc = tcgen05_prepare_b(dtype, src, bt, k, m, flags, t, &out->b_op, cnt.b_ready, &out->ready_target, side);
  cudaEventRecord(ev_join, side);
  out->forked = true;
  out->ready = cnt.b_ready;
  return rc;
}

int launch_tcgen05(int dtype, const GemmArgs &g, void *scratch, size_t scratch_bytes) {
  if (dtype != MM_DTYPE_FLOAT && dtype != MM_DTYPE_HALF && dtype != MM_DTYPE_UINT8 && dtype != MM_DTYPE_BFLOAT16) {
    return fail(MM_ERR_UNSUPPORTED, "tcgen05 path handles float, half, bfloat16 and uint8_t only");
  }
  if (g.tuning == nullptr) return fail(MM_ERR_INVALID, "tcgen05 launch without tuning");
  const Tuning &t = *g.tuning;
  if (g.dry_run) {
    cudaFuncAttributes attr;
    MM_CUDA_TRY(cudaFuncGetAttributes(&attr, round_tf32_kernel<true>));
    MM_CUDA_TRY(cudaFuncGetAttributes(&attr, round_tf32_kernel<false>));
    MM_CUDA_TRY(cudaFuncGetAttributes(&attr, prep_b_panels_kernel<true>));
    MM_CUDA_TRY(cudaFuncGetAttributes(&attr, prep_b_panels_kernel<false>));
    MM_CUDA_TRY(cudaFuncGetAttributes(&attr, transpose_prep_kernel<float, true>));
    MM_CUDA_TRY(cudaFuncGetAttributes(&attr, transpose_prep_kernel<__half, false>));
    MM_CUDA_TRY(cudaFuncGetAttributes(&attr, transpose_prep_kernel<unsigned char, false>));
    if (!get_encode_fn()) return fail(MM_ERR_CUDA, "cuTensorMapEncodeTiled entry point not available");
    return gemm_dispatch(dtype, nullptr, nullptr, nullptr, g.n, g.k, g.m, g.flags, t, nullptr, nullptr, 0, true, g.stream,
                         g.batch, g.accumulate);
  }
  if (scratch_bytes < tcgen05_scratch_bytes(dtype, g.n, g.k, g.m, g.flags, t, g.batch)) {
    return fail(MM_ERR_INVALID, "tcgen05 scratch too small");
  }
  unsigned char *sp = static_cast<unsigned char *>(scratch);
  void *aprep = sp + tcgen05_bt_bytes(dtype, g.k, g.m, g.flags, t, g.batch.b_copies());
  const Tcgen05Counters cnt = tcgen05_counters(scratch, scratch_bytes);
  BSource src;
  src.b = g.b;
  PreparedB pb;
  const void *a_op = nullptr;
  const HalfScratch hs = tcgen05_half_scratch(scratch, scratch_bytes, dtype, g.n, g.k, g.m, g.flags, t, g.batch);
  if (hs.fits_b) MM_CUDA_TRY(cudaMemsetAsync(hs.fits_b, 1, hs.flag_bytes, g.stream));
  int rc = tcgen05_prepare_b_async(dtype, src, nullptr, scratch, scratch_bytes, g.k, g.m, g.flags, t, g.stream,
                                   g.side_stream, g.ev_fork, g.ev_join, &pb, g.batch.b_copies(), hs.b, hs.fits_b);
  if (rc == MM_OK) {
    rc = tcgen05_prepare_a(dtype, g.a, aprep, g.n, g.k, g.flags, t, &a_op, g.stream, g.batch.a_copies(), hs.a,
                           hs.fits_a);
  }
  if (rc == MM_OK && g.agree != nullptr) rc = (*g.agree)(hs.fits_a, g.stream);
  if (rc == MM_OK && g.ev_prep_done) cudaEventRecord(g.ev_prep_done, g.stream);
  if (rc == MM_OK) {
    rc = tcgen05_gemm(dtype, a_op, pb.b_op, g.c, g.n, g.k, g.m, g.flags, t, cnt.tile_sync, pb.ready, pb.ready_target,
                      g.stream, g.batch, g.accumulate, hs.operands());
  }
  if (pb.forked) cudaStreamWaitEvent(g.stream, g.ev_join, 0);
  return rc;
}

}
```

Baseline: 663,300.

## Fuse float A/B prep into one kernel with lazy fp32 writeback

Replaces the separate round/transpose prep kernels for float operands with a single combined kernel that prepares A and B tiles together. Each tile writes only a half-precision copy while the operands still look half-representable, and writes the fp32 copy once the fits flags have already settled. A follow-up completion kernel writes fp32 tiles still owed, using per-tile pending bytes. The aim is to cut prep memory traffic and launch count, at the cost of a second pass plus extra flag and pending bookkeeping.

After: 690,300, median of 6. 4.1% higher.

```diff
diff --git a/gemm_hls_b200/csrc/capi.cu b/gemm_hls_b200/csrc/capi.cu
--- a/gemm_hls_b200/csrc/capi.cu
+++ b/gemm_hls_b200/csrc/capi.cu
@@ -405,9 +405,18 @@
     mm::HalfScratch hs;
     if (path == kPathTcgen05) {
       hs = mm::tcgen05_half_scratch(ctx->scratch.ptr, ctx->scratch.bytes, dtype, rows, k, m, flags, t);
-      if (hs.fits_b) MM_CUDA_TRY(cudaMemsetAsync(hs.fits_b, 1, hs.flag_bytes, ctx->stream));
-      rc = mm::tcgen05_prepare_b_async(dtype, src, db, ctx->scratch.ptr, ctx->scratch.bytes, k, m, flags, t, ctx->stream,
-                                       ctx->side, ctx->ev_fork, ctx->ev_join, &pb, 1, hs.b, hs.fits_b);
+      if (hs.fits_b) {
+        MM_CUDA_TRY(cudaMemsetAsync(hs.fits_b, 1, hs.flag_bytes, ctx->stream));
+        if (bp.parts_dev != nullptr) rc = mm::gather_b_rows(src, db, es, k, m, ctx->stream);
+        if (rc == MM_OK) {
+          rc = mm::tcgen05_prepare_float(false, nullptr, 0, 0, db, rows, k, m, flags, t, mm::GemmBatch{},
+                                         ctx->scratch.ptr, ctx->scratch.bytes, ctx->stream);
+        }
+        pb.b_op = ctx->scratch.ptr;
+      } else {
+        rc = mm::tcgen05_prepare_b_async(dtype, src, db, ctx->scratch.ptr, ctx->scratch.bytes, k, m, flags, t,
+                                         ctx->stream, ctx->side, ctx->ev_fork, ctx->ev_join, &pb, 1);
+      }
       if (rc != MM_OK) return rc;
       aprep = static_cast<unsigned char *>(ctx->scratch.ptr) + mm::tcgen05_bt_bytes(dtype, k, m, flags, t);
     } else if (bp.parts_dev != nullptr) {
@@ -420,10 +429,15 @@
       const size_t r0 = size_t(i) * chunk_rows, nr = std::min<size_t>(chunk_rows, rows - r0);
       MM_CUDA_TRY(cudaStreamWaitEvent(ctx->stream, ev_a(i), 0));
       if (path != kPathTcgen05) return MM_OK;
+      if (hs.fits_a != nullptr) {
+        a_ops[i] = aprep + r0 * k * es;
+        return mm::tcgen05_prepare_float(false, da + (ta ? 0 : r0 * k * es), unsigned(r0), unsigned(nr), nullptr, rows,
+                                         k, m, flags, t, mm::GemmBatch{}, ctx->scratch.ptr, ctx->scratch.bytes,
+                                         ctx->stream);
+      }
       const size_t a_scale = (dtype == MM_DTYPE_FLOAT && (flags & MM_FLAG_TF32X3)) ? 3 : 1;
       return mm::tcgen05_prepare_a(dtype, da + (ta ? 0 : r0 * k * es), aprep + (ta ? 0 : r0 * k * es * a_scale),
-                                   unsigned(nr), k, flags, t, &a_ops[i], ctx->stream, 1,
-                                   hs.a ? static_cast<unsigned char *>(hs.a) + r0 * k * 2 : nullptr, hs.fits_a);
+                                   unsigned(nr), k, flags, t, &a_ops[i], ctx->stream, 1);
     };
     auto compute = [&](unsigned i) -> int {
       const size_t r0 = size_t(i) * chunk_rows, nr = std::min<size_t>(chunk_rows, rows - r0);
@@ -447,6 +461,10 @@
       for (unsigned i = 0; i < chunks && rc == MM_OK; ++i) rc = prepare(i);
     }
     if (rc == MM_OK && agree != nullptr) rc = (*agree)(hs.fits_a, ctx->stream);
+    if (rc == MM_OK && prepare_first) {
+      rc = mm::tcgen05_prepare_float(true, da, 0, rows, db, rows, k, m, flags, t, mm::GemmBatch{}, ctx->scratch.ptr,
+                                     ctx->scratch.bytes, ctx->stream);
+    }
     for (unsigned i = 0; i < chunks && rc == MM_OK; ++i) {
       if (!prepare_first) rc = prepare(i);
       if (rc == MM_OK) rc = compute(i);
diff --git a/gemm_hls_b200/csrc/common.cuh b/gemm_hls_b200/csrc/common.cuh
--- a/gemm_hls_b200/csrc/common.cuh
+++ b/gemm_hls_b200/csrc/common.cuh
@@ -89,6 +89,7 @@
 struct HalfScratch {
   void *a = nullptr, *b = nullptr;
   unsigned int *fits_a = nullptr, *fits_b = nullptr;
+  unsigned char *pending_a = nullptr, *pending_b = nullptr;
   size_t flag_bytes = 0;
   HalfOperands operands() const { return HalfOperands{a, b, fits_a, fits_b}; }
 };
@@ -110,7 +111,7 @@
 Tcgen05Counters tcgen05_counters(void *scratch, size_t scratch_bytes);
 int tcgen05_prepare_b(int dtype, const BSource &src, void *bt, unsigned k, unsigned m, int flags, const Tuning &t,
                       const void **b_op, unsigned int *ready, unsigned *ready_target, cudaStream_t stream,
-                      unsigned copies = 1, void *bt16 = nullptr, unsigned int *fits = nullptr);
+                      unsigned copies = 1);
 struct PreparedB {
   const void *b_op = nullptr;
   const unsigned int *ready = nullptr;
@@ -119,11 +120,12 @@
 };
 int tcgen05_prepare_b_async(int dtype, const BSource &src, void *local_b, void *scratch, size_t scratch_bytes,
                             unsigned k, unsigned m, int flags, const Tuning &t, cudaStream_t stream, cudaStream_t side,
-                            cudaEvent_t ev_fork, cudaEvent_t ev_join, PreparedB *out, unsigned copies = 1,
-                            void *bt16 = nullptr, unsigned int *fits = nullptr);
+                            cudaEvent_t ev_fork, cudaEvent_t ev_join, PreparedB *out, unsigned copies = 1);
 int tcgen05_prepare_a(int dtype, const void *a, void *aprep, unsigned rows, unsigned k, int flags, const Tuning &t,
-                      const void **a_op, cudaStream_t stream, unsigned copies = 1, void *aprep16 = nullptr,
-                      unsigned int *fits = nullptr);
+                      const void **a_op, cudaStream_t stream, unsigned copies = 1);
+int tcgen05_prepare_float(bool complete, const void *a, unsigned row0, unsigned rows, const void *b, unsigned n,
+                          unsigned k, unsigned m, int flags, const Tuning &t, const GemmBatch &batch, void *scratch,
+                          size_t scratch_bytes, cudaStream_t stream);
 int tcgen05_gemm(int dtype, const void *a_op, const void *b_op, void *c, unsigned rows, unsigned k, unsigned m,
                  int flags, const Tuning &t, unsigned int *tile_sync, const unsigned int *b_ready,
                  unsigned b_ready_target, cudaStream_t stream, const GemmBatch &batch = GemmBatch{},
diff --git a/gemm_hls_b200/csrc/gemm_tcgen05.cu b/gemm_hls_b200/csrc/gemm_tcgen05.cu
--- a/gemm_hls_b200/csrc/gemm_tcgen05.cu
+++ b/gemm_hls_b200/csrc/gemm_tcgen05.cu
@@ -29,14 +29,11 @@
   return *reinterpret_cast<const uint32_t *>(&h);
 }
 
-template <bool HALF>
 __global__ void __launch_bounds__(256)
-round_tf32_kernel(const float4 *__restrict__ src, float4 *__restrict__ dst, size_t count4, uint2 *__restrict__ dst16,
-                  unsigned int *__restrict__ fits) {
+round_tf32_kernel(const float4 *__restrict__ src, float4 *__restrict__ dst, size_t count4) {
   src += size_t(blockIdx.y) * count4;
   dst += size_t(blockIdx.y) * count4;
   const size_t stride = size_t(gridDim.x) * blockDim.x;
-  bool fit = true;
   for (size_t i = size_t(blockIdx.x) * blockDim.x + threadIdx.x; i < count4; i += stride) {
     float4 v = src[i];
     v.x = round_tf32(v.x);
@@ -44,14 +41,202 @@
     v.z = round_tf32(v.z);
     v.w = round_tf32(v.w);
     dst[i] = v;
-    if constexpr (HALF) {
-      dst16[size_t(blockIdx.y) * count4 + i] = make_uint2(half2_bits(v.x, v.y), half2_bits(v.z, v.w));
-      fit = fit && tf32_fits_half(__float_as_uint(v.x)) && tf32_fits_half(__float_as_uint(v.y)) &&
-            tf32_fits_half(__float_as_uint(v.z)) && tf32_fits_half(__float_as_uint(v.w));
-    }
-  }
-  if constexpr (HALF) {
-    if (__syncthreads_or(!fit) && threadIdx.x == 0) fits[blockIdx.y] = 0u;
+  }
+}
+
+constexpr int FP_TILE = 64;
+constexpr int FP_THREADS = 256;
+
+struct FloatPrepOperand {
+  const float *src = nullptr;
+  float *dst = nullptr;
+  __half *dst16 = nullptr;
+  unsigned int *fits = nullptr;
+  const unsigned int *partner = nullptr;
+  uint32_t partner_stride = 0;
+  const unsigned int *other = nullptr;
+  uint32_t other_count = 0;
+  unsigned char *pending = nullptr;
+  uint32_t src_rows = 0, src_cols = 0, tiles_c = 0, items_per_copy = 0, items = 0;
+  bool transpose = false;
+  bool vec = false;
+};
+struct FloatPrepArgs {
+  FloatPrepOperand op[2];
+};
+
+struct FloatItemSmem {
+  float tile[FP_TILE][FP_TILE + 1];
+  int settled;
+};
+
+__device__ __forceinline__ bool settled_now(const FloatPrepOperand &o, uint32_t copy) {
+  const volatile unsigned int *own = o.fits;
+  if (own[copy] == 0u) return true;
+  const volatile unsigned int *partner = o.partner;
+  return partner != nullptr && partner[copy * o.partner_stride] == 0u;
+}
+
+template <bool COMPLETE>
+__device__ __forceinline__ void float_item(const FloatPrepOperand &o, uint32_t item, FloatItemSmem &sm) {
+  const uint32_t t = threadIdx.x;
+  const uint32_t copy = item / o.items_per_copy;
+  const uint32_t tile_i = item - copy * o.items_per_copy;
+  const uint32_t r0 = tile_i / o.tiles_c * FP_TILE, c0 = tile_i % o.tiles_c * FP_TILE;
+  const size_t base = size_t(copy) * o.src_rows * o.src_cols;
+  const float *src = o.src + base;
+  float v[16];
+  bool fit = true;
+  if (!o.transpose) {
+#pragma unroll
+    for (int j = 0; j < 2; ++j) {
+      const uint32_t q = t + FP_THREADS * j, r = r0 + q / 8, c = c0 + 8 * (q % 8);
+      float4 x = make_float4(0.f, 0.f, 0.f, 0.f), y = x;
+      if (r < o.src_rows && c < o.src_cols) {
+        const float4 *p = reinterpret_cast<const float4 *>(src + size_t(r) * o.src_cols + c);
+        x = p[0];
+        y = p[1];
+      }
+      v[8 * j + 0] = x.x; v[8 * j + 1] = x.y; v[8 * j + 2] = x.z; v[8 * j + 3] = x.w;
+      v[8 * j + 4] = y.x; v[8 * j + 5] = y.y; v[8 * j + 6] = y.z; v[8 * j + 7] = y.w;
+    }
+  } else {
+#pragma unroll
+    for (int j = 0; j < 4; ++j) {
+      const uint32_t f = t + FP_THREADS * j, r = r0 + f / 16, c = c0 + 4 * (f % 16);
+      float4 x = make_float4(0.f, 0.f, 0.f, 0.f);
+      if (r < o.src_rows) {
+        const float *p = src + size_t(r) * o.src_cols + c;
+        if (o.vec) {
+          if (c < o.src_cols) x = *reinterpret_cast<const float4 *>(p);
+        } else {
+          if (c + 0 < o.src_cols) x.x = p[0];
+          if (c + 1 < o.src_cols) x.y = p[1];
+          if (c + 2 < o.src_cols) x.z = p[2];
+          if (c + 3 < o.src_cols) x.w = p[3];
+        }
+      }
+      v[4 * j + 0] = x.x; v[4 * j + 1] = x.y; v[4 * j + 2] = x.z; v[4 * j + 3] = x.w;
+    }
+  }
+#pragma unroll
+  for (int e = 0; e < 16; ++e) {
+    v[e] = round_tf32(v[e]);
+    if (!COMPLETE) fit = fit && tf32_fits_half(__float_as_uint(v[e]));
+  }
+  if (o.transpose) {
+#pragma unroll
+    for (int j = 0; j < 4; ++j) {
+      const uint32_t f = t + FP_THREADS * j, r = f / 16, c = 4 * (f % 16);
+#pragma unroll
+      for (int e = 0; e < 4; ++e) sm.tile[r][c + e] = v[4 * j + e];
+    }
+  }
+  if (!COMPLETE && t == 0) sm.settled = settled_now(o, copy);
+  __syncthreads();
+  const bool settled = COMPLETE || sm.settled;
+  float *dst = o.dst + base;
+  __half *dst16 = o.dst16 + base;
+  const uint32_t ld = o.transpose ? o.src_rows : o.src_cols;
+  if (!o.transpose) {
+#pragma unroll
+    for (int j = 0; j < 2; ++j) {
+      const uint32_t q = t + FP_THREADS * j, r = r0 + q / 8, c = c0 + 8 * (q % 8);
+      if (r >= o.src_rows || c >= o.src_cols) continue;
+      const size_t off = size_t(r) * ld + c;
+      const float *w = v + 8 * j;
+      if (settled) {
+        reinterpret_cast<float4 *>(dst + off)[0] = make_float4(w[0], w[1], w[2], w[3]);
+        reinterpret_cast<float4 *>(dst + off)[1] = make_float4(w[4], w[5], w[6], w[7]);
+      } else {
+        *reinterpret_cast<uint4 *>(dst16 + off) =
+            make_uint4(half2_bits(w[0], w[1]), half2_bits(w[2], w[3]), half2_bits(w[4], w[5]), half2_bits(w[6], w[7]));
+      }
+    }
+  } else if (settled) {
+#pragma unroll
+    for (int j = 0; j < 4; ++j) {
+      const uint32_t idx = t + FP_THREADS * j, m = idx % 4 + 4 * (idx / 64), g = idx / 4 % 16;
+      if (c0 + m >= o.src_cols || r0 + 4 * g >= o.src_rows) continue;
+      float4 x;
+      x.x = sm.tile[4 * g + 0][m];
+      x.y = sm.tile[4 * g + 1][m];
+      x.z = sm.tile[4 * g + 2][m];
+      x.w = sm.tile[4 * g + 3][m];
+      *reinterpret_cast<float4 *>(dst + size_t(c0 + m) * ld + r0 + 4 * g) = x;
+    }
+  } else {
+#pragma unroll
+    for (int j = 0; j < 2; ++j) {
+      const uint32_t idx = t + FP_THREADS * j, m = idx % 8 + 8 * (idx / 64), g = idx / 8 % 8;
+      if (c0 + m >= o.src_cols || r0 + 8 * g >= o.src_rows) continue;
+      float x[8];
+#pragma unroll
+      for (int e = 0; e < 8; ++e) x[e] = sm.tile[8 * g + e][m];
+      *reinterpret_cast<uint4 *>(dst16 + size_t(c0 + m) * ld + r0 + 8 * g) =
+          make_uint4(half2_bits(x[0], x[1]), half2_bits(x[2], x[3]), half2_bits(x[4], x[5]), half2_bits(x[6], x[7]));
+    }
+  }
+  const int misfit = __syncthreads_or(!settled && !fit);
+  if (!COMPLETE && t == 0) {
+    if (settled) o.pending[item] = 0;
+    else if (misfit) o.fits[copy] = 0u;
+  }
+}
+
+__global__ void __launch_bounds__(FP_THREADS)
+prep_float_operands_kernel(const FloatPrepArgs args) {
+  __shared__ FloatItemSmem sm;
+  const uint32_t items0 = args.op[0].items, total = items0 + args.op[1].items;
+  for (uint32_t item = blockIdx.x; item < total; item += gridDim.x) {
+    if (item < items0) float_item<false>(args.op[0], item, sm);
+    else float_item<false>(args.op[1], item - items0, sm);
+  }
+}
+
+__device__ __forceinline__ bool read_on_tf32(const FloatPrepOperand &o, uint32_t copy, bool any_other_zero) {
+  if (o.fits[copy] == 0u) return true;
+  return o.partner != nullptr ? o.partner[copy * o.partner_stride] == 0u : any_other_zero;
+}
+
+__global__ void __launch_bounds__(FP_THREADS)
+complete_tf32_kernel(const FloatPrepArgs args) {
+  __shared__ FloatItemSmem sm;
+  __shared__ uint32_t owed[FP_THREADS];
+  __shared__ uint32_t owed_count;
+  const uint32_t t = threadIdx.x;
+  auto any_zero = [t](const FloatPrepOperand &o) {
+    bool z = false;
+    if (o.items != 0 && o.partner == nullptr) {
+      for (uint32_t w = t; w < o.other_count; w += FP_THREADS) z = z || o.other[w] == 0u;
+    }
+    return __syncthreads_or(z) != 0;
+  };
+  const bool zero0 = any_zero(args.op[0]), zero1 = any_zero(args.op[1]);
+  const uint32_t items0 = args.op[0].items, total = items0 + args.op[1].items;
+  if (t == 0) owed_count = 0;
+  __syncthreads();
+  for (size_t first = blockIdx.x; first < total; first += size_t(FP_THREADS) * gridDim.x) {
+    const size_t slot = first + size_t(t) * gridDim.x;
+    if (slot < total) {
+      const uint32_t item = uint32_t(slot);
+      const bool second = item >= items0;
+      const FloatPrepOperand &o = second ? args.op[1] : args.op[0];
+      const uint32_t local = second ? item - items0 : item;
+      if (read_on_tf32(o, local / o.items_per_copy, second ? zero1 : zero0) && o.pending[local] != 0) {
+        owed[atomicAdd(&owed_count, 1u)] = item;
+      }
+    }
+    __syncthreads();
+    const uint32_t count = owed_count;
+    for (uint32_t j = 0; j < count; ++j) {
+      const uint32_t it = owed[j];
+      if (it < items0) float_item<true>(args.op[0], it, sm);
+      else float_item<true>(args.op[1], it - items0, sm);
+    }
+    __syncthreads();
+    if (t == 0) owed_count = 0;
+    __syncthreads();
   }
 }
 
@@ -119,19 +304,9 @@
   }
 }
 
-template <typename T, bool ROUND>
-__device__ __forceinline__ T prep_value(T x) {
-  return x;
-}
-template <>
-__device__ __forceinline__ float prep_value<float, true>(float x) {
-  return round_tf32(x);
-}
-
-template <typename T, bool ROUND>
+template <typename T>
 __global__ void __launch_bounds__(256)
-transpose_prep_kernel(const T *__restrict__ src, T *__restrict__ dst, uint32_t src_rows,
-                      uint32_t src_cols, __half *__restrict__ dst16, unsigned int *__restrict__ fits) {
+transpose_prep_kernel(const T *__restrict__ src, T *__restrict__ dst, uint32_t src_rows, uint32_t src_cols) {
   constexpr int TILE = 64;
   constexpr int PAD = (sizeof(T) >= 4) ? 1 : 2;
   __shared__ T tile[TILE][TILE + PAD];
@@ -144,24 +319,13 @@
 #pragma unroll 4
   for (int i = y; i < TILE; i += 4) {
     const uint32_t r = r0 + i, c = c0 + x;
-    if (r < src_rows && c < src_cols) tile[i][x] = prep_value<T, ROUND>(src[size_t(r) * src_cols + c]);
+    if (r < src_rows && c < src_cols) tile[i][x] = src[size_t(r) * src_cols + c];
   }
   __syncthreads();
-  bool fit = true;
 #pragma unroll 4
   for (int i = y; i < TILE; i += 4) {
     const uint32_t c = c0 + i, r = r0 + x;
-    if (c < src_cols && r < src_rows) {
-      const T v = tile[x][i];
-      dst[size_t(c) * src_rows + r] = v;
-      if constexpr (ROUND) {
-        dst16[size_t(blockIdx.z) * src_rows * src_cols + size_t(c) * src_rows + r] = __float2half_rn(v);
-        fit = fit && tf32_fits_half(__float_as_uint(v));
-      }
-    }
-  }
-  if constexpr (ROUND) {
-    if (__syncthreads_or(!fit) && threadIdx.x == 0) fits[blockIdx.z] = 0u;
+    if (c < src_cols && r < src_rows) dst[size_t(c) * src_rows + r] = tile[x][i];
   }
 }
 
@@ -233,29 +397,20 @@
 
 size_t align_up(size_t x, size_t a) { return (x + a - 1) / a * a; }
 
-template <typename T, bool ROUND>
+template <typename T>
 void launch_transpose(const void *src, void *dst, uint32_t src_rows, uint32_t src_cols, cudaStream_t stream,
-                      unsigned copies, void *dst16 = nullptr, unsigned int *fits = nullptr) {
+                      unsigned copies) {
   dim3 grid((src_cols + 63) / 64, (src_rows + 63) / 64, copies);
-  transpose_prep_kernel<T, ROUND><<<grid, 256, 0, stream>>>(static_cast<const T *>(src), static_cast<T *>(dst),
-                                                           src_rows, src_cols, static_cast<__half *>(dst16), fits);
-}
-
-int launch_round(const void *src, void *dst, size_t count4, unsigned copies, void *dst16, unsigned int *fits,
-                 cudaStream_t stream) {
+  transpose_prep_kernel<T><<<grid, 256, 0, stream>>>(static_cast<const T *>(src), static_cast<T *>(dst), src_rows,
+                                                     src_cols);
+}
+
+int launch_round(const void *src, void *dst, size_t count4, unsigned copies, cudaStream_t stream) {
   const int blocks = int(std::min<size_t>((count4 + 255) / 256, size_t(num_sms()) * 16));
   const dim3 grid(std::max(blocks, 1), copies);
-  const float4 *s = static_cast<const float4 *>(src);
-  float4 *d = static_cast<float4 *>(dst);
-  if (dst16 != nullptr) {
-    MM_CUDA_TRY(cudaFuncSetAttribute(round_tf32_kernel<true>, cudaFuncAttributePreferredSharedMemoryCarveout,
-                                     cudaSharedmemCarveoutMaxShared));
-    round_tf32_kernel<true><<<grid, 256, 0, stream>>>(s, d, count4, static_cast<uint2 *>(dst16), fits);
-  } else {
-    MM_CUDA_TRY(cudaFuncSetAttribute(round_tf32_kernel<false>, cudaFuncAttributePreferredSharedMemoryCarveout,
-                                     cudaSharedmemCarveoutMaxShared));
-    round_tf32_kernel<false><<<grid, 256, 0, stream>>>(s, d, count4, nullptr, nullptr);
-  }
+  MM_CUDA_TRY(cudaFuncSetAttribute(round_tf32_kernel, cudaFuncAttributePreferredSharedMemoryCarveout,
+                                   cudaSharedmemCarveoutMaxShared));
+  round_tf32_kernel<<<grid, 256, 0, stream>>>(static_cast<const float4 *>(src), static_cast<float4 *>(dst), count4);
   return MM_OK;
 }
 
@@ -308,8 +463,11 @@
   if (dtype != MM_DTYPE_FLOAT && !(flags & MM_FLAG_TRANSPOSED_A)) return 0;
   return align_up(size_t(a_copies) * n * k * elem_bytes(dtype) * (split3(dtype, flags) ? 3 : 1), 1024);
 }
-size_t fits_bytes(const GemmBatch &batch) {
-  return align_up(size_t(batch.a_copies() + batch.b_copies()) * sizeof(unsigned int), 1024);
+uint32_t float_items(unsigned rows, unsigned cols) { return ceil_div(rows, FP_TILE) * ceil_div(cols, FP_TILE); }
+size_t fits_bytes(unsigned n, unsigned k, unsigned m, const GemmBatch &batch) {
+  return align_up(size_t(batch.a_copies() + batch.b_copies()) * sizeof(unsigned int) +
+                      size_t(batch.b_copies()) * float_items(k, m) + size_t(batch.a_copies()) * float_items(n, k),
+                  1024);
 }
 
 size_t tcgen05_bt_bytes(int dtype, unsigned k, unsigned m, int flags, const Tuning &t, unsigned b_copies) {
@@ -322,7 +480,7 @@
                              const GemmBatch &batch) {
   size_t bytes = TAIL_BYTES + tcgen05_bt_bytes(dtype, k, m, flags, t, batch.b_copies());
   bytes += a_copy_bytes(dtype, n, k, flags, batch.a_copies());
-  if (half_copies(dtype, flags, t)) bytes += align_up(size_t(batch.a_copies()) * n * k * 2, 1024) + fits_bytes(batch);
+  if (half_copies(dtype, flags, t)) bytes += align_up(size_t(batch.a_copies()) * n * k * 2, 1024) + fits_bytes(n, k, m, batch);
   return bytes;
 }
 
@@ -334,9 +492,11 @@
   const size_t bt = tcgen05_bt_bytes(dtype, k, m, flags, t, batch.b_copies());
   h.b = sp + b_copy_bytes(dtype, k, m, flags, batch.b_copies());
   h.a = sp + bt + a_copy_bytes(dtype, n, k, flags, batch.a_copies());
-  h.flag_bytes = fits_bytes(batch);
+  h.flag_bytes = fits_bytes(n, k, m, batch);
   h.fits_b = reinterpret_cast<unsigned int *>(sp + scratch_bytes - TAIL_BYTES - h.flag_bytes);
   h.fits_a = h.fits_b + batch.b_copies();
+  h.pending_b = reinterpret_cast<unsigned char *>(h.fits_a + batch.a_copies());
+  h.pending_a = h.pending_b + size_t(batch.b_copies()) * float_items(k, m);
   return h;
 }
 
@@ -347,7 +507,7 @@
 
 int tcgen05_prepare_b(int dtype, const BSource &src, void *bt, unsigned k, unsigned m, int flags, const Tuning &t,
                       const void **b_op, unsigned int *ready, unsigned *ready_target, cudaStream_t stream,
-                      unsigned copies, void *bt16, unsigned int *fits) {
+                      unsigned copies) {
   *b_op = bt;
   if (ready_target) *ready_target = 0;
   const bool parts = src.src != nullptr;
@@ -360,7 +520,7 @@
       return MM_OK;
     }
     if (!in_place && !parts && ready == nullptr) {
-      const int rc = launch_round(src.b, bt, size_t(k) * m / 4, 1, nullptr, nullptr, stream);
+      const int rc = launch_round(src.b, bt, size_t(k) * m / 4, 1, stream);
       if (rc != MM_OK) return rc;
       MM_CUDA_TRY(cudaGetLastError());
       return MM_OK;
@@ -382,22 +542,19 @@
     dim3 grid((m + 63) / 64, (k + 63) / 64, copies);
     split3_transpose_kernel<true><<<grid, 256, 0, stream>>>(static_cast<const float *>(b), static_cast<float *>(bt), k, m);
   } else if (dtype == MM_DTYPE_FLOAT) {
-    if (t.tf32_no_round()) {
-      launch_transpose<float, false>(b, bt, k, m, stream, copies);
-    } else {
-      launch_transpose<float, true>(b, bt, k, m, stream, copies, bt16, fits);
-    }
+    if (!t.tf32_no_round()) return fail(MM_ERR_INVALID, "float's rounded operands come from tcgen05_prepare_float");
+    launch_transpose<float>(b, bt, k, m, stream, copies);
   } else if (dtype == MM_DTYPE_UINT8) {
-    launch_transpose<unsigned char, false>(b, bt, k, m, stream, copies);
+    launch_transpose<unsigned char>(b, bt, k, m, stream, copies);
   } else {
-    launch_transpose<__half, false>(b, bt, k, m, stream, copies);
+    launch_transpose<__half>(b, bt, k, m, stream, copies);
   }
   MM_CUDA_TRY(cudaGetLastError());
   return MM_OK;
 }
 
 int tcgen05_prepare_a(int dtype, const void *a, void *aprep, unsigned rows, unsigned k, int flags, const Tuning &t,
-                      const void **a_op, cudaStream_t stream, unsigned copies, void *aprep16, unsigned int *fits) {
+                      const void **a_op, cudaStream_t stream, unsigned copies) {
   const bool transposed = (flags & MM_FLAG_TRANSPOSED_A) != 0;
   const size_t all_rows = size_t(copies) * rows;
   *a_op = a;
@@ -414,22 +571,87 @@
     }
     *a_op = aprep;
   } else if (dtype == MM_DTYPE_FLOAT) {
+    if (!t.tf32_no_round()) return fail(MM_ERR_INVALID, "float's rounded operands come from tcgen05_prepare_float");
     if (transposed) {
-      if (t.tf32_no_round()) {
-        launch_transpose<float, false>(a, aprep, k, rows, stream, copies);
-      } else {
-        launch_transpose<float, true>(a, aprep, k, rows, stream, copies, aprep16, fits);
-      }
+      launch_transpose<float>(a, aprep, k, rows, stream, copies);
       *a_op = aprep;
-    } else if (!t.tf32_no_round()) {
-      const int rc = launch_round(a, aprep, size_t(rows) * k / 4, copies, aprep16, fits, stream);
-      if (rc != MM_OK) return rc;
-      *a_op = aprep;
     }
   } else if (transposed) {
-    if (dtype == MM_DTYPE_UINT8) launch_transpose<unsigned char, false>(a, aprep, k, rows, stream, copies);
-    else launch_transpose<__half, false>(a, aprep, k, rows, stream, copies);
+    if (dtype == MM_DTYPE_UINT8) launch_transpose<unsigned char>(a, aprep, k, rows, stream, copies);
+    else launch_transpose<__half>(a, aprep, k, rows, stream, copies);
     *a_op = aprep;
+  }
+  MM_CUDA_TRY(cudaGetLastError());
+  return MM_OK;
+}
+
+namespace {
+FloatPrepOperand float_operand(const void *src, float *dst, __half *dst16, unsigned src_rows, unsigned src_cols,
+                               unsigned copies, bool transpose, unsigned int *fits, unsigned char *pending) {
+  FloatPrepOperand o;
+  o.src = static_cast<const float *>(src);
+  o.dst = dst;
+  o.dst16 = dst16;
+  o.fits = fits;
+  o.pending = pending;
+  o.src_rows = src_rows;
+  o.src_cols = src_cols;
+  o.tiles_c = ceil_div(src_cols, FP_TILE);
+  o.items_per_copy = float_items(src_rows, src_cols);
+  o.items = copies * o.items_per_copy;
+  o.transpose = transpose;
+  o.vec = src_cols % 4 == 0;
+  return o;
+}
+
+int float_prep_grid(const void *kernel, uint32_t items) {
+  MM_CUDA_TRY(cudaFuncSetAttribute(kernel, cudaFuncAttributePreferredSharedMemoryCarveout,
+                                   cudaSharedmemCarveoutMaxShared));
+  int per_sm = 0;
+  MM_CUDA_TRY(cudaOccupancyMaxActiveBlocksPerMultiprocessor(&per_sm, kernel, FP_THREADS, 0));
+  return int(std::max<uint32_t>(1u, std::min<uint32_t>(items, uint32_t(std::max(per_sm, 1) * num_sms()))));
+}
+}
+
+int tcgen05_prepare_float(bool complete, const void *a, unsigned row0, unsigned rows, const void *b, unsigned n,
+                          unsigned k, unsigned m, int flags, const Tuning &t, const GemmBatch &batch, void *scratch,
+                          size_t scratch_bytes, cudaStream_t stream) {
+  const HalfScratch hs = tcgen05_half_scratch(scratch, scratch_bytes, MM_DTYPE_FLOAT, n, k, m, flags, t, batch);
+  if (hs.fits_a == nullptr) return fail(MM_ERR_INVALID, "tcgen05_prepare_float: float on the default datapath only");
+  if (row0 % FP_TILE != 0) return fail(MM_ERR_INVALID, "tcgen05_prepare_float: A's first row must be a multiple of 64");
+  unsigned char *sp = static_cast<unsigned char *>(scratch);
+  const bool shared_a = batch.count > 1 && batch.shared_a, shared_b = batch.count > 1 && batch.shared_b;
+  FloatPrepArgs args;
+  if (b != nullptr) {
+    FloatPrepOperand &o = args.op[0];
+    o = float_operand(b, reinterpret_cast<float *>(sp), static_cast<__half *>(hs.b), k, m, batch.b_copies(), true,
+                      hs.fits_b, hs.pending_b);
+    o.partner = shared_b ? nullptr : hs.fits_a;
+    o.partner_stride = shared_a ? 0 : 1;
+    o.other = hs.fits_a;
+    o.other_count = batch.a_copies();
+  }
+  if (a != nullptr) {
+    const bool transposed = (flags & MM_FLAG_TRANSPOSED_A) != 0;
+    if (transposed && (row0 != 0 || rows != n)) return fail(MM_ERR_INVALID, "A stored K x N is prepared whole");
+    const size_t first = size_t(row0) * k;
+    float *aprep = reinterpret_cast<float *>(sp + tcgen05_bt_bytes(MM_DTYPE_FLOAT, k, m, flags, t, batch.b_copies()));
+    FloatPrepOperand &o = args.op[1];
+    o = float_operand(a, aprep + first, static_cast<__half *>(hs.a) + first, transposed ? k : rows,
+                      transposed ? rows : k, batch.a_copies(), transposed, hs.fits_a,
+                      hs.pending_a + size_t(row0 / FP_TILE) * ceil_div(k, FP_TILE));
+    o.partner = shared_a ? nullptr : hs.fits_b;
+    o.partner_stride = shared_b ? 0 : 1;
+    o.other = hs.fits_b;
+    o.other_count = batch.b_copies();
+  }
+  const uint32_t items = args.op[0].items + args.op[1].items;
+  if (complete) {
+    const int grid = float_prep_grid(reinterpret_cast<const void *>(complete_tf32_kernel), items);
+    complete_tf32_kernel<<<grid, FP_THREADS, 0, stream>>>(args);
+  } else {
+    const int grid = float_prep_grid(reinterpret_cast<const void *>(prep_float_operands_kernel), items);
+    prep_float_operands_kernel<<<grid, FP_THREADS, 0, stream>>>(args);
   }
   MM_CUDA_TRY(cudaGetLastError());
   return MM_OK;
@@ -473,29 +695,27 @@
 
 int tcgen05_prepare_b_async(int dtype, const BSource &src, void *local_b, void *scratch, size_t scratch_bytes,
                             unsigned k, unsigned m, int flags, const Tuning &t, cudaStream_t stream, cudaStream_t side,
-                            cudaEvent_t ev_fork, cudaEvent_t ev_join, PreparedB *out, unsigned copies, void *bt16,
-                            unsigned int *fits) {
+                            cudaEvent_t ev_fork, cudaEvent_t ev_join, PreparedB *out, unsigned copies) {
   *out = PreparedB{};
   const bool in_place = tcgen05_b_in_place(dtype, flags, t);
   const bool parts = src.src != nullptr;
   if (copies != 1) {
     if (parts) return fail(MM_ERR_UNSUPPORTED, "batched calls take B from one array");
-    return tcgen05_prepare_b(dtype, src, scratch, k, m, flags, t, &out->b_op, nullptr, nullptr, stream, copies, bt16,
-                             fits);
+    return tcgen05_prepare_b(dtype, src, scratch, k, m, flags, t, &out->b_op, nullptr, nullptr, stream, copies);
   }
   if (parts && !tcgen05_b_mn(dtype, flags, t)) {
     int rc = gather_b_rows(src, local_b, elem_bytes(dtype), k, m, stream);
     if (rc != MM_OK) return rc;
     BSource whole;
     whole.b = local_b;
-    return tcgen05_prepare_b(dtype, whole, scratch, k, m, flags, t, &out->b_op, nullptr, nullptr, stream, 1, bt16, fits);
+    return tcgen05_prepare_b(dtype, whole, scratch, k, m, flags, t, &out->b_op, nullptr, nullptr, stream, 1);
   }
   void *bt = in_place ? local_b : scratch;
   const Tcgen05Counters cnt = tcgen05_counters(scratch, scratch_bytes);
   const unsigned panels = ceil_div(m, unsigned(t.block_n()));
   const bool overlap = side != nullptr && t.b_overlap() != 0 && tcgen05_b_mn(dtype, flags, t) && (!in_place || parts) &&
                        panels <= B_READY_BYTES / sizeof(unsigned int);
-  if (!overlap) return tcgen05_prepare_b(dtype, src, bt, k, m, flags, t, &out->b_op, nullptr, nullptr, stream, 1, bt16, fits);
+  if (!overlap) return tcgen05_prepare_b(dtype, src, bt, k, m, flags, t, &out->b_op, nullptr, nullptr, stream, 1);
   MM_CUDA_TRY(cudaMemsetAsync(cnt.b_ready, 0, panels * sizeof(unsigned int), stream));
   MM_CUDA_TRY(cudaEventRecord(ev_fork, stream));
   MM_CUDA_TRY(cudaStreamWaitEvent(side, ev_fork, 0));
@@ -514,13 +734,13 @@
   const Tuning &t = *g.tuning;
   if (g.dry_run) {
     cudaFuncAttributes attr;
-    MM_CUDA_TRY(cudaFuncGetAttributes(&attr, round_tf32_kernel<true>));
-    MM_CUDA_TRY(cudaFuncGetAttributes(&attr, round_tf32_kernel<false>));
+    MM_CUDA_TRY(cudaFuncGetAttributes(&attr, round_tf32_kernel));
     MM_CUDA_TRY(cudaFuncGetAttributes(&attr, prep_b_panels_kernel<true>));
     MM_CUDA_TRY(cudaFuncGetAttributes(&attr, prep_b_panels_kernel<false>));
-    MM_CUDA_TRY(cudaFuncGetAttributes(&attr, transpose_prep_kernel<float, true>));
-    MM_CUDA_TRY(cudaFuncGetAttributes(&attr, transpose_prep_kernel<__half, false>));
-    MM_CUDA_TRY(cudaFuncGetAttributes(&attr, transpose_prep_kernel<unsigned char, false>));
+    MM_CUDA_TRY(cudaFuncGetAttributes(&attr, prep_float_operands_kernel));
+    MM_CUDA_TRY(cudaFuncGetAttributes(&attr, complete_tf32_kernel));
+    MM_CUDA_TRY(cudaFuncGetAttributes(&attr, transpose_prep_kernel<__half>));
+    MM_CUDA_TRY(cudaFuncGetAttributes(&attr, transpose_prep_kernel<unsigned char>));
     if (!get_encode_fn()) return fail(MM_ERR_CUDA, "cuTensorMapEncodeTiled entry point not available");
     return gemm_dispatch(dtype, nullptr, nullptr, nullptr, g.n, g.k, g.m, g.flags, t, nullptr, nullptr, 0, true, g.stream,
                          g.batch, g.accumulate);
@@ -536,14 +756,23 @@
   PreparedB pb;
   const void *a_op = nullptr;
   const HalfScratch hs = tcgen05_half_scratch(scratch, scratch_bytes, dtype, g.n, g.k, g.m, g.flags, t, g.batch);
-  if (hs.fits_b) MM_CUDA_TRY(cudaMemsetAsync(hs.fits_b, 1, hs.flag_bytes, g.stream));
-  int rc = tcgen05_prepare_b_async(dtype, src, nullptr, scratch, scratch_bytes, g.k, g.m, g.flags, t, g.stream,
-                                   g.side_stream, g.ev_fork, g.ev_join, &pb, g.batch.b_copies(), hs.b, hs.fits_b);
-  if (rc == MM_OK) {
-    rc = tcgen05_prepare_a(dtype, g.a, aprep, g.n, g.k, g.flags, t, &a_op, g.stream, g.batch.a_copies(), hs.a,
-                           hs.fits_a);
+  int rc = MM_OK;
+  if (hs.fits_b) {
+    MM_CUDA_TRY(cudaMemsetAsync(hs.fits_b, 1, hs.flag_bytes, g.stream));
+    pb.b_op = scratch;
+    a_op = aprep;
+    rc = tcgen05_prepare_float(false, g.a, 0, g.n, g.b, g.n, g.k, g.m, g.flags, t, g.batch, scratch, scratch_bytes,
+                               g.stream);
+  } else {
+    rc = tcgen05_prepare_b_async(dtype, src, nullptr, scratch, scratch_bytes, g.k, g.m, g.flags, t, g.stream,
+                                 g.side_stream, g.ev_fork, g.ev_join, &pb, g.batch.b_copies());
+    if (rc == MM_OK) rc = tcgen05_prepare_a(dtype, g.a, aprep, g.n, g.k, g.flags, t, &a_op, g.stream, g.batch.a_copies());
   }
   if (rc == MM_OK && g.agree != nullptr) rc = (*g.agree)(hs.fits_a, g.stream);
+  if (rc == MM_OK && hs.fits_b) {
+    rc = tcgen05_prepare_float(true, g.a, 0, g.n, g.b, g.n, g.k, g.m, g.flags, t, g.batch, scratch, scratch_bytes,
+                               g.stream);
+  }
   if (rc == MM_OK && g.ev_prep_done) cudaEventRecord(g.ev_prep_done, g.stream);
   if (rc == MM_OK) {
     rc = tcgen05_gemm(dtype, a_op, pb.b_op, g.c, g.n, g.k, g.m, g.flags, t, cnt.tile_sync, pb.ready, pb.ready_target,
```
